# linhthi/BLISS-GNN

Hardware: AMD Instinct MI355X
Metric: steps/sec (train step: sample_blocks + gather + SAGE fwd/bwd + Adam + exp3), reddit-like (higher is better)
Workload: dtype bf16

## Files before the change

bliss_gnn_amd/_engine.py:

```python
import ctypes as C
import os
from typing import NamedTuple

import numpy as np
import torch

from . import _lib
from .graph import Block, Graph

_CHUNK = 1024
_CAP_ERRS = 1 | 2 | 4 | 8 | 64


def _ptr(t):
    return 0 if t is None else t.data_ptr()


def _stream():
    return torch.cuda.current_stream().cuda_stream


def _up8(n):
    return (int(n) + 7) & ~7

# ... 52 lines not shown
    "wlabor": _Kind("node", prob="any", entry="bliss_wlabor_layer", tail=lambda d, row: (_dep(d),) + _prob_args(d, row), p_out=True,
                    scratch=lambda e, s, b: e._scratch_grown("_wl_scr", "bliss_wlabor_scratch_bytes", s, b)),
}


class _Draw(NamedTuple):
    state: object = None
    prob: dict = None
    layer_dependency: bool = False
    iterations: int = 0


_LayerOut = NamedTuple("_LayerOut", [(name, object) for name in
                                     "indptr src dst pos eid w q kept_nid node_prob counts t_indptr t_edge".split()])


def _exact_b(rule, Eg, s, f):
    return int(min(rule.b_limit or Eg, s * f))


def layer_caps(kind, V, Eg, S0, fanouts, have=None):
    rule = KINDS[kind]
    if have is not None and len(have) != len(fanouts):
        have = None
    if have is not None and have[0]["S"] >= S0:
        if rule.k_slack is None:
            return have
        caps = [dict(c) for c in have]
    else:
        caps, s = [], int(S0)
        for f in fanouts:
            f = int(f)
            if rule.family == "layer":
                k = min(V, int(1.25 * (f + s)) + 64)
                b = int(min(Eg, max(1 << 16, 48 * k)))
            elif f < 0:
                k, b = V, int(min(Eg, max(1 << 16, 48 * s)))
            else:
                b = _exact_b(rule, Eg, s, f) if rule.b_limit is not None else int(min(Eg, 2 * s * f + 4096))
                k = int(min(V, s + min(b, Eg)))
            caps.append(dict(S=s, C=V, K=k, B=b))
            s = k
        if have is not None:
            caps = [{k: max(a.get(k, 0), b[k]) for k in b} for a, b in zip(have, caps)]
    if rule.k_slack is not None:
        for n, f in enumerate(fanouts):
            caps[n]["K"] = max(caps[n]["K"], min(V, int(f) + caps[n]["S"] + rule.k_slack))
            if n + 1 < len(caps):
                caps[n + 1]["S"] = max(caps[n + 1]["S"], caps[n]["K"])
    return have if caps == have else caps


def static_caps(kind, V, Eg, S0, fanouts, max_sizes, k_margin=1.5, b_margin=3.0):
    rule = KINDS[kind]
    caps, s = [], int(S0)
    for n, f in enumerate(fanouts):
        k = min(V, int(k_margin * max_sizes[n]["K"]) + 256)
        if rule.k_slack == 0:
            k = min(V, int(f) + s)
        b = int(min(Eg, int(b_margin * max_sizes[n]["B"]) + 4096))
        if rule.b_limit is not None and int(f) >= 0:
            b = _exact_b(rule, Eg, s, int(f))
        e = int(min(Eg, int(1.5 * max_sizes[n].get("E", Eg)) + 65536))
        x = int(min(b, int(1.5 * max_sizes[n]["B"]) + 2048))
        caps.append(dict(S=s, C=V, K=k, B=b, E=e, X=x))
        s = k
    return caps


def _parse_counts(counts_host, L):
    raw = counts_host.numpy().tobytes()
    cnts = [_lib.LayerCounts.from_buffer_copy(raw[40 * n: 40 * n + 40]) for n in range(L)]
    bad = 0
    for c in cnts:
        bad |= c.err
    return cnts, bad


class _LayerWs:

    def __init__(self, dev, cap_s, cap_c):
        self.cap_s, self.cap_c = cap_s, cap_c
        self.seg_ptr = torch.empty(cap_s + 1, dtype=torch.int32, device=dev)
        self.seed_acc = torch.empty(72 * cap_s + 64, dtype=torch.uint8, device=dev)
        self.cand_nid = torch.empty(cap_c, dtype=torch.int32, device=dev)
        self.new_id = torch.empty(cap_c, dtype=torch.int32, device=dev)
        self.p = torch.empty(cap_c, dtype=torch.bfloat16, device=dev)
        self.P = torch.empty(cap_c, dtype=torch.bfloat16, device=dev)
        self.uniforms = torch.empty(cap_c, dtype=torch.float32, device=dev)
        self.keys = torch.empty(cap_c, dtype=torch.float32, device=dev)
        self.draw_scr = torch.zeros(int(_lib.lib.bliss_multinomial_draw_scratch_bytes(cap_c)) // 4, dtype=torch.int32, device=dev)
        self.rdraw_scr = None
        self.src_cnt = None
        self.tr_temp = None


class DrawState:

    def __init__(self, seed, step, device):
        self.seed = int(seed) & ((1 << 64) - 1)
        self.step_dev = torch.tensor([int(step)], dtype=torch.int64, device=device)

    def step(self):
        return int(self.step_dev.item())


class LayerEngine:

    def __init__(self, g: Graph, kind="stream"):
        if kind not in KINDS:
            raise ValueError("kind must be one of %s, not %r" % (", ".join(KINDS), kind))
        if g.device.type != "cuda":
            raise RuntimeError("bliss_gnn_amd samples on the GPU only; move the graph with g.to('cuda') "
                               "(the reference's --data-cpu/--use-uva modes are out of scope)")
        self.g = g
        dev = g.device
        V = g.num_nodes()
        self.V, self.Eg = V, g.num_edges()
        if self.Eg >= 2 ** 31:
            raise RuntimeError("int32 edge positions: graphs with >= 2^31 edges are not supported")
        self.scratch_sets = 2
        self._sets = {}
        self.first_pos = torch.full((V,), -1, dtype=torch.int32, device=dev)
        self.acc_p2 = torch.zeros(V, dtype=torch.int64, device=dev)
        self.c_graph = _lib.Graph(g.indptr.data_ptr(), g.indices.data_ptr(), _ptr(g.eid), V, self.Eg)
        self.flags = torch.zeros(16, dtype=torch.int32, device=dev)
        self.fs_ticket = torch.zeros(1, dtype=torch.int32, device=dev)
        self.fuse_scale = os.environ.get("BLISS_FUSE_SCALE", "1") != "0"
        self.flag_err = torch.zeros(1, dtype=torch.int32, device=dev)
        self.n_bins = 0
        for nb in ((int(os.environ["BLISS_NBINS"]),) if os.environ.get("BLISS_NBINS") else (256, 1024)):
            if -(-V // nb) * 12 <= 64 * 1024:
                self.n_bins = nb
                break
        if os.environ.get("BLISS_BINS", "1") == "0" or self.Eg > 2048 * 4096 * 32:
            self.n_bins = 0
        self._bins = None
        self.hist = torch.zeros(32768, dtype=torch.int32, device=dev)
        self.mt_dev = torch.empty(626, dtype=torch.int32, device=dev)
        self.mt_host = torch.empty(626, dtype=torch.int32).pin_memory()
        self.mt_back = torch.empty(626, dtype=torch.int32).pin_memory()
        self._static = {}
        self._static_draw = {}
        self.kind = kind
        self._nr_scr = None
        self._nb_scr = None
        self._wn_scr = None
        self._lb_scr = None
        self._li_scr = None
        self._wl_scr = None
        self._wl_p = {}
        self._slot_bufs, self._slot_counts, self._slot_counts_host = {}, {}, {}
        self.caps = None
        self.ws = None
        self.counts_host = None
        self.retries = 0

    def _set(self, n):
        i = n % self.scratch_sets
        if i not in self._sets:
            dev, V = self.g.device, self.V
            local_id = torch.full((V,), -1, dtype=torch.int32, device=dev)
            self._sets[i] = dict(local_id=local_id, kept_map=torch.full((V,), -1, dtype=torch.int32, device=dev),
                                 span_seg=torch.zeros(self.Eg // 256 + 2, dtype=torch.int32, device=dev),
                                 chunk_cnt=torch.empty(max(self.Eg, V) // _CHUNK + 2, dtype=torch.int32, device=dev),
                                 kept_rec=None, span_cnt=None,
                                 c_maps=_lib.NodeMaps(local_id.data_ptr(), self.first_pos.data_ptr(), self.acc_p2.data_ptr()))
# ... 514 lines not shown
```

bliss_gnn_amd/_lib.py:

```python
import ctypes as C
import os

_HERE = os.path.dirname(os.path.abspath(__file__))
LIB_PATH = os.path.join(_HERE, "libbliss_gnn.so")

EINVAL = -1
MODE_BANDIT, MODE_LADIES, MODE_UNIFORM_NODES, MODE_PARTIALS = 0, 1, 4, 8
NR_MAX_FANOUT = 1024
WN_RAW, WN_EXP3 = 0, 1

ERR_BITS = {
    1: "frontier larger than 2^31-1 edges",
    2: "candidate capacity exceeded / seed id out of range",
    4: "kept-node capacity exceeded",
    8: "block-edge capacity exceeded",
    16: "non-finite or negative weight reached an exact reduction",
    32: "exact sum left its fixed-point range",
    64: "seed capacity exceeded",
    128: "random stream ran short / generator made no progress",
    256: "a cross-stream flag never came (bliss_flag_wait timed out)",
}


class Graph(C.Structure):
# ... 178 lines not shown
class BlockOut(C.Structure):
    _fields_ = [("indptr", C.c_void_p), ("src", C.c_void_p), ("dst", C.c_void_p), ("pos", C.c_void_p),
                ("eid", C.c_void_p), ("edge_weights", C.c_void_p), ("q_ij", C.c_void_p), ("t_indptr", C.c_void_p),
                ("t_edge", C.c_void_p), ("t_scratch", C.c_void_p), ("cap_b", C.c_int32)]


_P, _I32, _I64, _F, _D = C.c_void_p, C.c_int32, C.c_int64, C.c_float, C.c_double

SIGNATURES = {
    "bliss_layer_counts_bytes": [],
    "bliss_frontier_prob": [C.POINTER(Graph), C.POINTER(NodeMaps), _P, _P, _I32, _P, _I32, C.c_int, _F, _F, _I64, C.POINTER(LayerWs), _P],
    "bliss_rng_stream_begin": [_P, _P, _P, _P, _I32, _P],
    "bliss_rng_stream_wait": [_P, _P, _P, C.c_int, _I32, _P],
    "bliss_rng_stream_end": [_P, _P, _P, _I32, _P, _P],
    "bliss_rng_stream_chain": [_P, _P, _P, _P, _I32, _P, _I32, _P, _P],
    "bliss_rng_stream_ready": [_P],
    "bliss_rng_prepare": [_I32, _P],
    "bliss_mt_jump_poly": [_I64, _P],
    "bliss_flag_wait": [_P, _P, _P],
    "bliss_flag_set_spin_bound": [C.c_int64],
    "bliss_flag_raise": [_P, _P],
    "bliss_gather_rows": [_P, _I64, _P, _I32, _I32, _P, _I64, _P, _P],
    "bliss_exp3_apply_ranks": [C.POINTER(Exp3RankLists), _P, _P, _P, _P],
    "bliss_pack_lists": [C.POINTER(PackLists), _P, _P],
    "bliss_mt19937_uniform": [_P, _P, _I32, _P, _I32, _P],
    "bliss_poisson_select": [C.POINTER(LayerWs), _I32, _D, _P, _P, _P, C.c_int, _I32, _I64, _P],
    "bliss_poisson_select_keyed": [C.POINTER(LayerWs), _I32, _D, C.c_uint64, _P, _I32, C.c_int, _I64, _P],
    "bliss_multinomial_select": [C.POINTER(LayerWs), _P, _I32, _P],
    "bliss_multinomial_draw": [_P, _P, _P, _I32, _I32, _P, C.c_uint64, _P, _I32, C.c_int, _P, _P, _P, _P],
    "bliss_multinomial_select_marked": [C.POINTER(LayerWs), _P],
    "bliss_neighbor_layer": [C.POINTER(Graph), _P, _I32, _P, _I32, _I32, _P, C.c_uint64, _P, _I32, C.c_int, C.POINTER(LayerWs),
                             C.POINTER(BlockOut), _P, _P],
    "bliss_wneighbor_layer": [C.POINTER(Graph), _P, _I32, _P, _I32, _I32, _P, C.c_uint64, _P, _I32, C.c_int, _I32, _P, _F, _F, _P,
                              C.POINTER(LayerWs), C.POINTER(BlockOut), _P, _P],
    "bliss_neighbor_replace_layer": [C.POINTER(Graph), _P, _I32, _P, _I32, _I32, _P, C.c_uint64, _P, _I32, C.c_int, _P, _P,
                                     C.POINTER(LayerWs), C.POINTER(BlockOut), _P, _P],
    "bliss_multinomial_draw_replace": [_P, _P, _I32, _I32, _P, C.c_uint64, _P, _I32, C.c_int, _P, _P, _P, _P],
    "bliss_labor_layer": [C.POINTER(Graph), _P, _I32, _P, _I32, _I32, _P, C.c_uint64, _P, _I32, C.c_int, C.c_int, C.POINTER(LayerWs),
                          C.POINTER(BlockOut), _P, _P],
    "bliss_labor_is_layer": [C.POINTER(Graph), _P, _I32, _P, _I32, _I32, _P, C.c_uint64, _P, _I32, C.c_int, C.c_int, _I32,
                             C.POINTER(LayerWs), C.POINTER(BlockOut), _P, _P],
    "bliss_wlabor_layer": [C.POINTER(Graph), _P, _I32, _P, _I32, _I32, _P, C.c_uint64, _P, _I32, C.c_int, C.c_int, _I32, _P, _F, _F,
                           C.POINTER(LayerWs), C.POINTER(BlockOut), _P, _P, _P],
    "bliss_tile_gemm": [C.POINTER(TileGemm), C.POINTER(TileGemm), _P],
    "bliss_cross_entropy": [_P, _I64, _P, _I32, _I32, _P, _P, _I64, _P, _P, _P, _P],
    "bliss_cross_entropy_sum": [_P, _I64, _P, _I64, _P, _P, _I32, _I32, _P, _P, _I64, _P, _P, _P, _P],
    "bliss_cross_entropy_masked": [_P, _I64, _P, _I64, _P, _I32, _P, _I32, _I32, _P, _F, _I32, _P, _P, _I64, _P, _P, _P, _P],
    "bliss_cross_entropy_live": [_P, _I64, _P, _I64, _P, _P, _I32, _P, _I32, _P, _P, _I64, _P, _P, _P, _P],
    "bliss_bce_logits_live": [_P, _I64, _P, _I64, _P, _P, _I32, _P, _I32, _P, _P, _I64, _P, _P, _P, _P],
    "bliss_bce_logits": [_P, _I64, _P, _I32, _I32, _P, _P, _I64, _P, _P, _P, _P],
    "bliss_bce_logits_sum": [_P, _I64, _P, _I64, _P, _P, _I32, _I32, _P, _P, _I64, _P, _P, _P, _P],
    "bliss_bce_logits_masked": [_P, _I64, _P, _I64, _P, _I32, _P, _I32, _I32, _P, _F, _I32, _P, _P, _I64, _P, _P, _P, _P],
    "bliss_f1_multiclass": [_P, _I64, _I32, _P, _P, _P, _I32, _P, _I32, _P, _I32, _P, _P, _P],
    "bliss_f1_multilabel": [_P, _I64, _I32, _P, _P, _P, _I32, _P, _I32, _P, _I32, _P, _P, _P],
    "bliss_adam_step": [C.POINTER(AdamTensors), _P, _F, _F, _F, _F, _P],
    "bliss_step_ledger_bytes": [C.c_int],
    "bliss_step_ledger": [C.c_int, _P, C.c_int, _P, C.c_int, C.POINTER(C.c_int32), _D, _D, _P, _P],
    "bliss_batch_stats": [C.c_int, _P, C.c_int, _P, _P],
    "bliss_cand_importance": [_P, _I32, C.c_int, _P, _P, _P],
    "bliss_poisson_scale": [_P, _P, _I32, _D, _P, _P],
    "bliss_keyed_select": [_P, _P, _P, _I32, _P, C.c_uint64, C.c_uint64, _I32, _P, _P, _P],
    "bliss_exp3_normalize_global": [_P, _I64, _P, _P, _P, _P, _P],
    "bliss_build_block": [C.POINTER(Graph), C.POINTER(NodeMaps), _P, _P, _I32, C.c_int, _F, _F, _I64, C.POINTER(LayerWs), C.POINTER(BlockOut), _P],
    "bliss_normalized_edata": [C.POINTER(Graph), _P, _P],
    "bliss_embed_norm": [_P, _I32, _I32, _I64, _P, _P],
    "bliss_spmm_fwd": [_P, _P, _P, _P, _P, _I64, _I32, _P, _I32, _I32, C.c_int, _P, _I64, C.c_int, _P, _P],
    "bliss_spmm_bwd": [_P, _P, _P, _P, _P, _P, _P, _I64, _I32, _P, _I32, _I32, C.c_int, _P, _I64, C.c_int, _P, _P],
    "bliss_block_transpose": [_P, _P, _I32, _I32, _I32, _P, _P, _P, _I64, _P],
    "bliss_spmm_chunk_edges": [_I32],
    "bliss_sage_epilogue_fwd": [_P, _I64, _P, _I64, _I32, _I32, _F, C.c_uint32, _P, _P, _I64, _P, _P],
    "bliss_sage_epilogue_bwd": [_P, _I64, _P, _I64, _I32, _I32, _F, _P, _I64, _P],
    "bliss_gat_chunk_edges": [],
    "bliss_graph_prepare": [_P, _P, _I64, _I32, C.c_int, _P, _P, _P, _P, _P, _P, _I64, _P],
    "bliss_exp3_update": [C.POINTER(Graph), _P, _P, _P, _P, _P, _P, _P, _P, _P, _P, _P, _P, _I32, _P, _I32, _F, _P, _P, C.c_int, _P, _P],
    "bliss_exp3_step": [C.POINTER(Graph), _P, C.POINTER(Exp3Block), _I32, _F, _P, _P],
    "bliss_exp3_normalize_global_rows": [C.POINTER(Exp3Block), _I32, _I64, _P, _I64, _P],
    "bliss_exp3_update_blocks": [C.POINTER(Graph), _P, C.POINTER(Exp3Block), _I32, _F, _P, _P],
    "bliss_exp3_apply": [_P, _P, _P, _P, _P, _I32, _P, _P],
    "bliss_exp3_normalize": [_P, _I64, _P, _P, _P, _P],
    "bliss_row_sum": [_P, _I64, _P, _P],
    "bliss_gat_logits": [_P, _P, _P, _I32, _P, _I64, _P, _I32, _I32, _F, _P, _P],
    "bliss_sage_dgrad": [C.POINTER(DGrad), _P],
    "bliss_sage_wgrad": [C.POINTER(WGrad), _I32, _P, _I64, _P],
    "bliss_gat_dgrad": [C.POINTER(DGrad), _P],
    "bliss_gat_glue_fwd": [C.POINTER(GatGlue), _P],
    "bliss_gat_glue_bwd": [C.POINTER(GatGlue), _P],
    "bliss_gat_head_mean": [_P, _I32, _I32, _P, _P, _P],
    "bliss_gcn_norms": [_P, _I32, _P, _I32, _P, _P, _P],
    "bliss_gcn_spmm_fwd": [_P, _P, _P, _P, _P, _P, _P, _I64, _I32, _P, _I32, _I32, _P, _I64, _P, _P],
    "bliss_gcn_spmm_bwd": [_P, _P, _P, _P, _P, _P, _P, _P, _I64, _I32, _P, _I32, _I32, _P, _I64, _P, _P],
    "bliss_gcn_db_chunk_rows": [],
    "bliss_gcn_epilogue_fwd": [C.POINTER(GcnEpilogue), _P],
    "bliss_gcn_epilogue_bwd": [C.POINTER(GcnEpilogue), _P],
    "bliss_gcn_infer_chunk_edges": [_I32],
    "bliss_gcn_infer_src_norms": [C.POINTER(GcnInfer), _P],
    "bliss_gcn_infer_spmm": [C.POINTER(GcnInfer), _P],
    "bliss_shard_local_seeds": [_P, _I32, _P, _I32, _I32, _I32, _P, _P, _P, _P, _P, _P],
    "bliss_shard_scatter_partials": [_P, _P, _P, _P, _P, _P, _P, _I32, _P, _P],
    "bliss_shard_zero_dense": [_P, _I32, _P],
    "bliss_shard_pack_rows": [_P, _P, _I32, _I32, _I32, _P, _I64, _I32, _P, _I64, _P],
    "bliss_shard_place_rows": [_P, _I64, _P, _P, _I32, _P, _I64, _I32, _I32, _P],
    "bliss_shard_take_rows": [_P, _I32, _I64, _I32, _P, _P, _I32, _P, _I64, _I32, _P],
    "bliss_shard_candidates": [_P, _I32, _I32, _P, _P, _P, _P, _P, _I32, _P, _P, _P],
    "bliss_shard_select_kept": [_P, _P, _P, _P, C.c_uint64, _P, _I32, _P, _I32, _P, _P, _P, _P, _P, _I32, _I32, _I32, _P, _P, _P, _I32, _P, _P, _P],
    "bliss_gat_fused_supported": [_I32, _I32],
    "bliss_gat_segment_edges": [],
    "bliss_gat_fused_stamps": [_P, _P],
    "bliss_gat_segments": [_P, _I32, _I32, _P, _P, _P, _P],
    "bliss_gat_fused_fwd": [C.POINTER(GatFused), _P],
    "bliss_gat_fused_bwd_dst": [C.POINTER(GatFused), _P, _P, _P, _P],
    "bliss_gat_infer_fwd": [C.POINTER(GatInfer), _P],
    "bliss_gat_rows_src_fused": [_P, _I32, _P, _P, _P, _P, _I32, _P, _P, _P, _I64, _P, _I64, _P, _I32, _I32, _F, _P, _I64, _P, _P],
    "bliss_gat_logits_f32": [_P, _P, _P, _I32, _P, _I64, _P, _I32, _I32, _F, _P, _P],
    "bliss_gat_edge_dot": [_P, _P, _P, _I32, _P, _I64, _P, _I64, _I32, _I32, _P, _P],
    "bliss_gat_edge_softmax": [_P, _I32, _P, _P, _I32, C.c_int, _P, _P],
    "bliss_gat_rows": [C.c_int, _P, _I32, _P, _P, _P, _P, _I32, _P, _P, _I64, _P, _I32, _I32, _F, _P, _I64, _P, _P, _P],
    "bliss_gat_alpha": [_P, _I32, _P, _P, _P, _P, _P],
    "bliss_prof_enable": [C.c_int],
    "bliss_prof_reset": [],
    "bliss_prof_read": [C.c_int, C.POINTER(C.c_double), C.POINTER(C.c_int64)],
    "bliss_prof_kernel_count": [],
}


SPECIAL_SIGNATURES = ("bliss_prof_kernel_name", "bliss_block_transpose_temp_bytes", "bliss_graph_prepare_capacity",
                      "bliss_graph_prepare_temp_bytes", "bliss_rng_stream_handle", "bliss_sage_wgrad_workspace",
                      "bliss_multinomial_draw_scratch_bytes", "bliss_neighbor_scratch_bytes", "bliss_wneighbor_scratch_bytes",
                      "bliss_labor_scratch_bytes", "bliss_labor_is_scratch_bytes", "bliss_wlabor_scratch_bytes",
                      "bliss_neighbor_replace_scratch_bytes", "bliss_multinomial_draw_replace_scratch_bytes")


def _load():
    if not os.path.exists(LIB_PATH):
        raise ImportError(
            f"{LIB_PATH} not found: build it with `python -c 'import __graft_entry__ as g; g.build()'` "
            "or `make -C bliss_gnn_amd/csrc`.  bliss_gnn_amd has no CPU or PyTorch fallback.")
    lib = C.CDLL(LIB_PATH)
    for name, argtypes in SIGNATURES.items():
        fn = getattr(lib, name)
        fn.argtypes = argtypes
        fn.restype = C.c_int
    lib.bliss_block_transpose_temp_bytes.argtypes = [_I32, _I32]
    lib.bliss_block_transpose_temp_bytes.restype = C.c_int64
    lib.bliss_sage_wgrad_workspace.argtypes = [C.POINTER(WGrad), _I32]
    lib.bliss_sage_wgrad_workspace.restype = C.c_int64
    for name in ("bliss_graph_prepare_capacity", "bliss_graph_prepare_temp_bytes"):
        getattr(lib, name).argtypes = [_I64, _I32, C.c_int]
        getattr(lib, name).restype = C.c_int64
    lib.bliss_multinomial_draw_scratch_bytes.argtypes = [_I32]
    lib.bliss_multinomial_draw_scratch_bytes.restype = C.c_int64
    lib.bliss_neighbor_scratch_bytes.argtypes = [_I32, _I32]
    lib.bliss_neighbor_scratch_bytes.restype = C.c_int64
    lib.bliss_wneighbor_scratch_bytes.argtypes = [_I32, _I32, _I64]
    lib.bliss_wneighbor_scratch_bytes.restype = C.c_int64
    lib.bliss_labor_scratch_bytes.argtypes = [_I32, _I32]
    lib.bliss_labor_scratch_bytes.restype = C.c_int64
    lib.bliss_labor_is_scratch_bytes.argtypes = [_I32, _I32, _I32]
    lib.bliss_labor_is_scratch_bytes.restype = C.c_int64
    lib.bliss_wlabor_scratch_bytes.argtypes = [_I32, _I32, _I32]
    lib.bliss_wlabor_scratch_bytes.restype = C.c_int64
    lib.bliss_neighbor_replace_scratch_bytes.argtypes = [_I32, _I32]
    lib.bliss_neighbor_replace_scratch_bytes.restype = C.c_int64
    lib.bliss_multinomial_draw_replace_scratch_bytes.argtypes = [_I32]
    lib.bliss_multinomial_draw_replace_scratch_bytes.restype = C.c_int64
    lib.bliss_rng_stream_handle.argtypes = []
    lib.bliss_rng_stream_handle.restype = C.c_int64
    lib.bliss_prof_kernel_name.argtypes = [C.c_int]
    lib.bliss_prof_kernel_name.restype = C.c_char_p
    assert lib.bliss_layer_counts_bytes() == C.sizeof(LayerCounts), "LayerCounts layout mismatch"
    assert all(lib.bliss_step_ledger_bytes(n) == C.sizeof(ledger_struct(n)) for n in range(1, LEDGER_MAX_LAYERS + 1)), \
        "step ledger layout mismatch"
    assert C.sizeof(BatchStats) == 32, "batch statistics layout mismatch"
    return lib


lib = _load()


def check(rc, what):
    if rc != 0:
        raise RuntimeError(f"{what} failed with code {rc}" + (" (invalid argument)" if rc == EINVAL else " (hipError_t)"))


def err_string(bits):
    return "; ".join(msg for b, msg in ERR_BITS.items() if bits & b) or "unknown"
```

bliss_gnn_amd/csrc/sage_bwd.hip:

```cpp
#include "common.cuh"
#include "bliss_gnn.h"
#include <cstdlib>

namespace {

typedef __bf16 bf16x8_t __attribute__((ext_vector_type(8)));
typedef short s16x4_t __attribute__((ext_vector_type(4)));
typedef short s16x8_t __attribute__((ext_vector_type(8)));
typedef float f32x16_t __attribute__((ext_vector_type(16)));
typedef uint32_t u32x4_a4 __attribute__((ext_vector_type(4), aligned(4)));

__device__ __forceinline__ s16x4_t lds_tr4(const bf16_t* p) {
  return __builtin_amdgcn_ds_read_tr16_b64_v4i16((__attribute__((address_space(3))) s16x4_t*)(p));
}
__device__ __forceinline__ bf16x8_t tr_frag(const bf16_t* img, int stride, int k0, int c0, int lane) {
  const int g = lane >> 4, i = lane & 15, q = i >> 2, p = i & 3;
  const bf16_t* a = img + (size_t)(k0 + 8 * (g >> 1) + q) * stride + c0 + 16 * (g & 1) + 4 * p;
  const s16x4_t lo = lds_tr4(a), hi = lds_tr4(a + 4 * (size_t)stride);
  s16x8_t v;
  v[0] = lo[0]; v[1] = lo[1]; v[2] = lo[2]; v[3] = lo[3]; v[4] = hi[0]; v[5] = hi[1]; v[6] = hi[2]; v[7] = hi[3];
  return __builtin_bit_cast(bf16x8_t, v);
}

__device__ __forceinline__ uint4 ld16(const bf16_t* p) {
// ... 41 lines not shown
    *reinterpret_cast<uint4*>(wl + (size_t)kr * DG_WSTRIDE + 8 * c8) = v;
  }
}

__device__ __forceinline__ void dg_product(const bf16_t* tile, int k, const bf16_t* __restrict__ w, long long w_stride, int N, int n0,
                                           bf16_t* wl, int tid, int lane, int wave, f32x16_t& acc) {
  const int st = dg_astride(k), kp = (k + 15) & ~15, r = lane & 31, h = lane >> 5;
  const int nslab = (kp + DG_SLAB - 1) / DG_SLAB;
  for (int sl = 0; sl < nslab; ++sl) {
    __syncthreads();
    dg_stage_w(w, w_stride, k, N, n0, sl, wl, tid);
    __syncthreads();
#pragma unroll
    for (int s = 0; s < DG_SLAB / 16; ++s) {
      const int ks = sl * DG_SLAB + 16 * s;
      if (ks < kp) {
        const bf16x8_t a = *reinterpret_cast<const bf16x8_t*>(tile + (size_t)r * st + ks + 8 * h);
        const bf16x8_t b = tr_frag(wl, DG_WSTRIDE, 16 * s, 32 * wave, lane);
        acc = __builtin_amdgcn_mfma_f32_32x32x16_bf16(a, b, acc, 0, 0, 0);
      }
    }
  }
}

__global__ void __launch_bounds__(DG_TPB) k_dgrad(DGrad p) {
  extern __shared__ __attribute__((aligned(16))) bf16_t dg_lds[];
  const int tid = threadIdx.x, wave = tid >> 6, lane = tid & 63;
  int M = p.m_bound;
  if (p.m_dev) { const int t = *p.m_dev; M = t < M ? t : M; }
  int M2 = p.k2 ? p.m2_bound : 0;
  if (p.k2 && p.m2_dev) { const int t = *p.m2_dev; M2 = t < M2 ? t : M2; }
  if (M2 > M) M2 = M;
  const int row0 = blockIdx.x * DG_M, n0 = blockIdx.y * 256, N = p.n;
  if (row0 >= p.m_bound) return;
  const bool pair_ok = (p.out_stride % 2 == 0) && (((uintptr_t)p.out) % 4 == 0) && (N % 2 == 0);
  if (row0 >= M) {
    for (int idx = tid; idx < DG_M * 256; idx += DG_TPB) {
      const int r = row0 + (idx >> 8), c = n0 + (idx & 255);
      if (r < p.m_bound && c < N) p.out[(long long)r * p.out_stride + c] = 0;
    }
    return;
  }
  const int s1 = dg_astride(p.k1), s2 = p.k2 ? dg_astride(p.k2) : 0;
  bf16_t* t1 = dg_lds;
  bf16_t* t2 = t1 + (size_t)DG_M * s1;
  bf16_t* wl = t2 + (size_t)DG_M * s2;
  dg_stage_a(p.a1, p.a1_stride, p.k1, row0, M, t1, tid);
  const bool second = p.k2 && row0 < M2;
  if (second) dg_stage_a(p.a2, p.a2_stride, p.k2, row0, M2, t2, tid);
  f32x16_t acc;
#pragma unroll
  for (int i = 0; i < 16; ++i) acc[i] = 0.f;
  dg_product(t1, p.k1, p.w1, p.w1_stride, N, n0, wl, tid, lane, wave, acc);
  if (second) dg_product(t2, p.k2, p.w2, p.w2_stride, N, n0, wl, tid, lane, wave, acc);
  __syncthreads();
  const int so = 256 + 8;
  bf16_t* ot = dg_lds;
  {
    const int col = 32 * wave + (lane & 31);
#pragma unroll
    for (int i = 0; i < 16; ++i) {
      const int lr = (i & 3) + 8 * (i >> 2) + 4 * (lane >> 5);
      ot[(size_t)lr * so + col] = (row0 + lr < M) ? f2bf(acc[i]) : (bf16_t)0;
    }
  }
  __syncthreads();
  for (int lr = wave; lr < DG_M; lr += DG_TPB / 64) {
    const int r = row0 + lr;
    if (r >= p.m_bound) break;
    const bf16_t* sh = ot + (size_t)lr * so;
    bf16_t* o = p.out + (long long)r * p.out_stride + n0;
    const int nn = min(256, N - n0);
    if (pair_ok && (n0 % 2 == 0)) { for (int c = lane * 2; c < nn; c += 128) *reinterpret_cast<uint32_t*>(o + c) = *reinterpret_cast<const uint32_t*>(sh + c); }
    else for (int c = lane; c < nn; c += 64) o[c] = sh[c];
  }
}

#define WG_TPB 512
#define WG_ROWS 32
#define WG_TN 128
#define WG_DSTRIDE (256 + 32)
#define WG_XSTRIDE (WG_TN + 32)
#define WG_MAX_PROBS 2

struct WGradProb {
  const bf16_t* d; long long d_stride; int n_out;
  const bf16_t* x; long long x_stride; int k_in;
  int rows_bound; const int* rows_dev;
  bf16_t* dw; long long dw_stride; bf16_t* db;
  int col_tiles, chunks, rows_per_chunk; long long part_off;
  int ldp;
  int wg_begin;
};
struct WGradLaunch { WGradProb p[WG_MAX_PROBS]; int n; };

struct WRegsB { uint4 d[2]; uint4 x; };

__device__ __forceinline__ void wg_load(WRegsB& g, const WGradProb& p, int r_lo, int r_hi, int c0, int tid, bool d_al, bool x_al) {
#pragma unroll
  for (int i = 0; i < 2; ++i) {
    const int idx = tid + i * WG_TPB, lr = idx >> 5, c8 = idx & 31, r = r_lo + lr, n = 8 * c8;
    g.d[i] = (r < r_hi) ? ld8_masked(p.d + (long long)r * p.d_stride + n, p.n_out - n, d_al) : make_uint4(0, 0, 0, 0);
  }
  {
    const int lr = tid >> 4, c8 = tid & 15, r = r_lo + lr, c = c0 + 8 * c8;
    g.x = (r < r_hi) ? ld8_masked(p.x + (long long)r * p.x_stride + c, p.k_in - c, x_al) : make_uint4(0, 0, 0, 0);
  }
}
__device__ __forceinline__ void wg_store(const WRegsB& g, bf16_t* dimg, bf16_t* ximg, int tid) {
#pragma unroll
  for (int i = 0; i < 2; ++i) {
    const int idx = tid + i * WG_TPB, lr = idx >> 5, c8 = idx & 31;
    *reinterpret_cast<uint4*>(dimg + (size_t)lr * WG_DSTRIDE + 8 * c8) = g.d[i];
  }
  *reinterpret_cast<uint4*>(ximg + (size_t)(tid >> 4) * WG_XSTRIDE + 8 * (tid & 15)) = g.x;
}

__global__ void __launch_bounds__(WG_TPB) k_wgrad(WGradLaunch L, float* __restrict__ part) {
  __shared__ __attribute__((aligned(16))) bf16_t dimg[WG_ROWS * WG_DSTRIDE];
  __shared__ __attribute__((aligned(16))) bf16_t ximg[WG_ROWS * WG_XSTRIDE];
  const int tid = threadIdx.x, wave = tid >> 6, lane = tid & 63;
  const int pi = (L.n > 1 && (int)blockIdx.x >= L.p[1].wg_begin) ? 1 : 0;
  const WGradProb& p = L.p[pi];
  const int w = (int)blockIdx.x - p.wg_begin;
  const int ct = w % p.col_tiles, ch = w / p.col_tiles;
  int R = p.rows_bound;
  if (p.rows_dev) { const int t = *p.rows_dev; R = t < R ? t : R; }
  const int r_lo = ch * p.rows_per_chunk, r_hi = min(R, r_lo + p.rows_per_chunk);
  if (r_lo >= r_hi) return;
  const int c0 = ct * WG_TN;
  const int wm = wave >> 1, wn = wave & 1;
  const int m0 = 64 * wm, nl0 = 64 * wn;
  const bool m_act = m0 < p.n_out;
  const bool bias = p.db != nullptr && ct == 0 && wn == 0;
  f32x16_t acc[2][2], accb[2];
#pragma unroll
  for (int a = 0; a < 2; ++a) {
#pragma unroll
    for (int i = 0; i < 16; ++i) { acc[a][0][i] = 0.f; acc[a][1][i] = 0.f; accb[a][i] = 0.f; }
  }
  s16x8_t ones_s;
#pragma unroll
  for (int j = 0; j < 8; ++j) ones_s[j] = (short)0x3f80;
  const bf16x8_t ones = __builtin_bit_cast(bf16x8_t, ones_s);
  const bool d_al = (p.d_stride % 2 == 0) && (((uintptr_t)p.d) % 4 == 0);
  const bool x_al = (p.x_stride % 2 == 0) && (((uintptr_t)p.x) % 4 == 0);
  WRegsB g;
  wg_load(g, p, r_lo, r_hi, c0, tid, d_al, x_al);
  for (int rs = r_lo; rs < r_hi; rs += WG_ROWS) {
    __syncthreads();
    wg_store(g, dimg, ximg, tid);
    if (rs + WG_ROWS < r_hi) wg_load(g, p, rs + WG_ROWS, r_hi, c0, tid, d_al, x_al);
    __syncthreads();
    if (m_act) {
#pragma unroll
      for (int ks = 0; ks < WG_ROWS; ks += 16) {
        const bf16x8_t a0 = tr_frag(dimg, WG_DSTRIDE, ks, m0, lane), a1 = tr_frag(dimg, WG_DSTRIDE, ks, m0 + 32, lane);
        const bf16x8_t b0 = tr_frag(ximg, WG_XSTRIDE, ks, nl0, lane), b1 = tr_frag(ximg, WG_XSTRIDE, ks, nl0 + 32, lane);
        acc[0][0] = __builtin_amdgcn_mfma_f32_32x32x16_bf16(a0, b0, acc[0][0], 0, 0, 0);
        acc[0][1] = __builtin_amdgcn_mfma_f32_32x32x16_bf16(a0, b1, acc[0][1], 0, 0, 0);
        acc[1][0] = __builtin_amdgcn_mfma_f32_32x32x16_bf16(a1, b0, acc[1][0], 0, 0, 0);
        acc[1][1] = __builtin_amdgcn_mfma_f32_32x32x16_bf16(a1, b1, acc[1][1], 0, 0, 0);
        if (bias) {
          accb[0] = __builtin_amdgcn_mfma_f32_32x32x16_bf16(a0, ones, accb[0], 0, 0, 0);
          accb[1] = __builtin_amdgcn_mfma_f32_32x32x16_bf16(a1, ones, accb[1], 0, 0, 0);
        }
      }
    }
  }
  if (!m_act) return;
  float* pt = part + p.part_off + (long long)ch * 256 * p.ldp;
#pragma unroll
  for (int a = 0; a < 2; ++a) {
#pragma unroll
    for (int i = 0; i < 16; ++i) {
      const int n = m0 + 32 * a + (i & 3) + 8 * (i >> 2) + 4 * (lane >> 5);
      float* row = pt + (long long)n * p.ldp;
      row[c0 + nl0 + (lane & 31)] = acc[a][0][i];
      row[c0 + nl0 + 32 + (lane & 31)] = acc[a][1][i];
      if (bias && (lane & 31) == 0) row[p.col_tiles * WG_TN] = accb[a][i];
    }
  }
}

__global__ void __launch_bounds__(256) k_wgrad_reduce(WGradLaunch L, const float* __restrict__ part) {
  const int pi = blockIdx.y;
  const WGradProb& p = L.p[pi];
  int R = p.rows_bound;
  if (p.rows_dev) { const int t = *p.rows_dev; R = t < R ? t : R; }
  const int nch = R > 0 ? min(p.chunks, (R + p.rows_per_chunk - 1) / p.rows_per_chunk) : 0;
  const int q4 = (p.k_in + 3) / 4 + (p.db ? 1 : 0);
  const long long total = (long long)p.n_out * q4;
  const float* base = part + p.part_off;
  for (long long idx = (long long)blockIdx.x * 256 + threadIdx.x; idx < total; idx += (long long)gridDim.x * 256) {
    const int n = (int)(idx / q4), q = (int)(idx - (long long)n * q4);
    if (p.db && q == q4 - 1) {
      float s = 0.f;
      for (int c = 0; c < nch; ++c) s += base[((long long)c * 256 + n) * p.ldp + p.col_tiles * WG_TN];
      p.db[n] = f2bf(s);
      continue;
    }
    float4 s = make_float4(0.f, 0.f, 0.f, 0.f);
    for (int c = 0; c < nch; ++c) {
      const float4 v = *reinterpret_cast<const float4*>(base + ((long long)c * 256 + n) * p.ldp + 4 * q);
      s.x += v.x; s.y += v.y; s.z += v.z; s.w += v.w;
    }
    bf16_t* o = p.dw + (long long)n * p.dw_stride + 4 * q;
    const int left = p.k_in - 4 * q;
    o[0] = f2bf(s.x);
    if (left > 1) o[1] = f2bf(s.y);
    if (left > 2) o[2] = f2bf(s.z);
    if (left > 3) o[3] = f2bf(s.w);
  }
}

int wgrad_target_wgs() {
  static const int t = []() { const char* e = getenv("BLISS_WGRAD_WGS"); const int v = e ? atoi(e) : 0; return v > 0 ? v : 80; }();
  return t;
}

bool wgrad_plan(const bliss_wgrad_t* a, int n_probs, WGradLaunch* L, long long* floats, int* total_wgs) {
  if (n_probs < 1 || n_probs > WG_MAX_PROBS) return false;
  long long off = 0;
  int wgs = 0;
  int tiles_all = 0;
  for (int i = 0; i < n_probs; ++i) {
    if (!a[i].d || !a[i].x || !a[i].dw || a[i].n_out <= 0 || a[i].n_out > 256 || a[i].k_in <= 0 || a[i].rows_bound <= 0) return false;
    tiles_all += (a[i].k_in + WG_TN - 1) / WG_TN;
  }
  for (int i = 0; i < n_probs; ++i) {
    WGradProb& p = L->p[i];
    p.d = (const bf16_t*)a[i].d; p.d_stride = a[i].d_stride; p.n_out = a[i].n_out;
    p.x = (const bf16_t*)a[i].x; p.x_stride = a[i].x_stride; p.k_in = a[i].k_in;
    p.rows_bound = a[i].rows_bound; p.rows_dev = a[i].rows_dev;
    p.dw = (bf16_t*)a[i].dw; p.dw_stride = a[i].dw_stride; p.db = (bf16_t*)a[i].db;
    p.col_tiles = (a[i].k_in + WG_TN - 1) / WG_TN;
    int chunks = wgrad_target_wgs() / tiles_all;
    const int max_chunks = (a[i].rows_bound + 63) / 64;
    if (chunks > max_chunks) chunks = max_chunks;
    if (chunks < 1) chunks = 1;
    int rpc = (a[i].rows_bound + chunks - 1) / chunks;
    rpc = (rpc + WG_ROWS - 1) / WG_ROWS * WG_ROWS;
    chunks = (a[i].rows_bound + rpc - 1) / rpc;
    p.chunks = chunks; p.rows_per_chunk = rpc;
    p.ldp = p.col_tiles * WG_TN + 4;
    p.part_off = off;
    p.wg_begin = wgs;
    off += (long long)chunks * 256 * p.ldp;
    wgs += chunks * p.col_tiles;
  }
  L->n = n_probs;
  *floats = off;
  *total_wgs = wgs;
  return true;
}

int dgrad_launch(const bliss_dgrad_t* a, int k_max, void* stream) {
  if (!a || !a->a1 || !a->w1 || !a->out || a->k1 <= 0 || a->k1 > k_max || a->n <= 0 || a->m_bound <= 0) return BLISS_EINVAL;
  if (a->k2 < 0 || a->k2 > k_max || (a->k2 > 0 && (!a->a2 || !a->w2 || a->m2_bound <= 0))) return BLISS_EINVAL;
  DGrad p;
  p.a1 = (const bf16_t*)a->a1; p.a1_stride = a->a1_stride; p.w1 = (const bf16_t*)a->w1; p.w1_stride = a->w1_stride; p.k1 = a->k1;
  p.a2 = (const bf16_t*)a->a2; p.a2_stride = a->a2_stride; p.w2 = (const bf16_t*)a->w2; p.w2_stride = a->w2_stride; p.k2 = a->k2;
  p.m2_bound = a->m2_bound; p.m2_dev = a->m2_dev;
  p.m_bound = a->m_bound; p.m_dev = a->m_dev; p.n = a->n;
  p.out = (bf16_t*)a->out; p.out_stride = a->out_stride;
  const size_t stage = ((size_t)DG_M * (dg_astride(a->k1) + (a->k2 ? dg_astride(a->k2) : 0)) + (size_t)DG_SLAB * DG_WSTRIDE) * sizeof(bf16_t);
  const size_t outt = (size_t)DG_M * (256 + 8) * sizeof(bf16_t);
  const size_t lds = stage > outt ? stage : outt;
  if (lds > 160 * 1024) return BLISS_EINVAL;
  static size_t lds_set = 0;
  if (lds > lds_set) {
    if (hipFuncSetAttribute((const void*)k_dgrad, hipFuncAttributeMaxDynamicSharedMemorySize, (int)lds) != hipSuccess) return BLISS_EINVAL;
    lds_set = lds;
  }
  const dim3 grid((a->m_bound + DG_M - 1) / DG_M, (a->n + 255) / 256);
  k_dgrad<<<grid, DG_TPB, lds, (hipStream_t)stream>>>(p);
  return (int)hipGetLastError();
}

}

extern "C" {

int bliss_sage_dgrad(const bliss_dgrad_t* a, void* stream) { return dgrad_launch(a, 256, stream); }

int bliss_gat_dgrad(const bliss_dgrad_t* a, void* stream) { return dgrad_launch(a, 1024, stream); }

int64_t bliss_sage_wgrad_workspace(const bliss_wgrad_t* probs, int32_t n_probs) {
  WGradLaunch L;
  long long floats = 0;
  int wgs = 0;
  if (!probs || !wgrad_plan(probs, n_probs, &L, &floats, &wgs)) return -1;
  return (int64_t)floats;
}

int bliss_sage_wgrad(const bliss_wgrad_t* probs, int32_t n_probs, float* partials, int64_t partial_floats, void* stream) {
  WGradLaunch L;
  long long floats = 0;
  int wgs = 0;
  if (!probs || !partials || !wgrad_plan(probs, n_probs, &L, &floats, &wgs)) return BLISS_EINVAL;
  if (partial_floats < floats || (((uintptr_t)partials) % 16) != 0) return BLISS_EINVAL;
  hipStream_t st = (hipStream_t)stream;
  k_wgrad<<<wgs, WG_TPB, 0, st>>>(L, partials);
  int max_elems = 0;
  for (int i = 0; i < n_probs; ++i) { const int e = L.p[i].n_out * ((L.p[i].k_in + 3) / 4 + 1); if (e > max_elems) max_elems = e; }
  int gx = (max_elems + 255) / 256;
  if (gx > 1024) gx = 1024;
  k_wgrad_reduce<<<dim3(gx, n_probs), 256, 0, st>>>(L, partials);
  return (int)hipGetLastError();
}

}
```

bliss_gnn_amd/csrc/sampler.hip:

```cpp
#include "common.cuh"
#include "bliss_gnn.h"
#include "prof.h"
#include "edge_q.cuh"
#include "keyed_uniform.cuh"
#include <cstdlib>

#ifndef TPB
#define TPB 256
#endif
#define ITEMS 4
#define CHUNK (TPB * ITEMS)

namespace {

#define SPAN (64 * ITEMS)
#define SEG_ZERO_WGS 8
#define LONG_COL 1024
#define LONG_FIRST 4096

struct alignas(8) ColEnt {
  int k, n;
  long long p0;
};

struct EdgeAt {
  int k;
  int64_t pos;
  int src;
};

__device__ __forceinline__ EdgeAt decode(int base, int E, int S, const int* __restrict__ seg_ptr,
                                         const long long* __restrict__ col_base, const int* __restrict__ indices, int* k_hint) {
  EdgeAt r;
  const int e = base + lane_id();
  r.k = wave_segment(seg_ptr, S, base, k_hint);
  r.pos = 0; r.src = 0;
  if (e < E) {
    r.pos = col_base[r.k] + e;
    r.src = indices[r.pos];
  } else r.k = -1;
  return r;
}

struct SpanAt {
  int k[ITEMS];
  int64_t pos[ITEMS];
  int src[ITEMS];
};
__device__ __forceinline__ bool decode_span(int wbase, int E, int S, const int* __restrict__ seg_ptr,
                                            const long long* __restrict__ col_base, const int* __restrict__ indices, int k_hint,
                                            SpanAt& r) {
  k_hint = k_hint < 0 ? 0 : (k_hint < S ? k_hint : S - 1);
  if (!span_segments<ITEMS>(seg_ptr, S, wbase, E - 1, k_hint, r.k)) return false;
  long long cb[ITEMS];
#pragma unroll
  for (int j = 0; j < ITEMS; ++j) cb[j] = col_base[r.k[j]];
#pragma unroll
  for (int j = 0; j < ITEMS; ++j) {
    const int e = wbase + j * 64 + lane_id();
    r.pos[j] = cb[j] + (e < E ? e : E - 1);
    r.src[j] = indices[r.pos[j]];
  }
  return true;
}

__device__ __forceinline__ int chunk_wave_offset(int wave_total, int* sh4, int* chunk_total) {
  const int wave = threadIdx.x >> 6;
  __syncthreads();
  if (lane_id() == 0) sh4[wave] = wave_total;
  __syncthreads();
  int off = 0, tot = 0;
#pragma unroll
  for (int w = 0; w < TPB / 64; ++w) { const int v = sh4[w]; tot += v; if (w < wave) off += v; }
  *chunk_total = tot;
  return off;
}

__device__ __forceinline__ void seg_scan_body(const int64_t* __restrict__ indptr, const int* __restrict__ seeds,
                                              LayerCounts* cnt, int S_host, const int* __restrict__ S_dev, int cap_s,
                                              unsigned long long* __restrict__ seed_acc, int* __restrict__ seg_ptr,
                                              int* __restrict__ local_id, int num_nodes, int* __restrict__ src_cnt, int cap_k,
                                              int* __restrict__ bin_cursor, int n_bins, long long* __restrict__ col_base,
                                              int* __restrict__ span_seg, long long frontier_cap, int* entry_flag,
                                              int wg, int n_wgs, bool keep_sums, int* sh, int* st_sh, ColEnt* long_list = nullptr) {
  if (entry_flag && wg == 0 && threadIdx.x == 0) __hip_atomic_store(entry_flag, 1, __ATOMIC_RELEASE, __HIP_MEMORY_SCOPE_AGENT);
  __shared__ int sh_long[2];
  if (long_list && threadIdx.x < 2) sh_long[threadIdx.x] = 0;
  int S = S_host >= 0 ? S_host : *S_dev;
  int bad = 0;
  if (S > cap_s) { S = cap_s; bad |= BLISS_ERR_CAP_SEEDS; }
  if (wg > 0 || n_wgs == 1) {
    const int nz = n_wgs > 1 ? n_wgs - 1 : 1, bz = n_wgs > 1 ? wg - 1 : 0;
    const int t0 = bz * blockDim.x + threadIdx.x, step = nz * blockDim.x;
    for (int i = (keep_sums ? 2 * cap_s : 0) + t0; i < cap_s * 5; i += step) seed_acc[i] = 0ull;
    if (src_cnt) for (int i = t0; i <= cap_k; i += step) src_cnt[i] = 0;
    if (bin_cursor) for (int i = t0; i <= n_bins; i += step) bin_cursor[i] = 0;
    for (int k = t0; k < S; k += step) { const int s = seeds[k]; if (s >= 0 && s < num_nodes) local_id[s] = k; }
    if (n_wgs > 1) return;
  }
  long long run = 0;
  constexpr int G = 4;
  for (int base0 = 0; base0 < S; base0 += G * (int)blockDim.x) {
    int degs[G];
    long long cols[G];
#pragma unroll
    for (int i = 0; i < G; ++i) {
      const int k = base0 + i * (int)blockDim.x + threadIdx.x;
      degs[i] = 0; cols[i] = 0;
      if (k < S) {
        const int s = seeds[k];
        if (s < 0 || s >= num_nodes) { bad |= BLISS_ERR_CAP_CAND; }
        else {
          cols[i] = indptr[s];
          degs[i] = (int)(indptr[s + 1] - cols[i]);
        }
      }
    }
#pragma unroll
    for (int i = 0; i < G; ++i) {
      const int k = base0 + i * (int)blockDim.x + threadIdx.x;
      if (base0 + i * (int)blockDim.x >= S) break;
      const int deg = degs[i];
      int tot, ex = block_excl_scan(deg, sh, &tot);
      const long long start = run + ex;
      if (k < S) {
        seg_ptr[k] = (int)start;
        col_base[k] = deg > 0 ? cols[i] - start : 0;
      }
      if (long_list) {
        const bool is_long = k < S && deg > LONG_COL, is_first = is_long && deg > LONG_FIRST;
        const unsigned long long m_first = __ballot(is_first), m_rest = __ballot(is_long && !is_first);
        if (m_first | m_rest) {
          int b_first = 0, b_rest = 0;
          if (lane_id() == 0) {
            if (m_first) b_first = atomicAdd(&sh_long[0], __popcll(m_first));
            if (m_rest) b_rest = atomicAdd(&sh_long[1], __popcll(m_rest));
          }
          b_first = __shfl(b_first, 0); b_rest = __shfl(b_rest, 0);
          if (is_long) {
            const unsigned long long below = (1ull << lane_id()) - 1ull;
            const int slot = is_first ? b_first + __popcll(m_first & below) : cap_s - 1 - (b_rest + __popcll(m_rest & below));
            ColEnt ent; ent.k = k; ent.n = deg; ent.p0 = cols[i];
            long_list[slot] = ent;
          }
        }
      }
      if (run + tot <= frontier_cap) {
        st_sh[threadIdx.x] = (int)(k < S ? start : run + tot);
        __syncthreads();
        const long long sp_end = (run + tot + SPAN - 1) / SPAN;
        for (long long sp = (run + SPAN - 1) / SPAN + threadIdx.x; sp < sp_end; sp += blockDim.x) {
          const int p = (int)(sp * SPAN);
          int t = 0;
#pragma unroll
          for (int step = 512; step >= 1; step >>= 1) if (st_sh[t + step] <= p) t += step;
          span_seg[sp] = base0 + i * (int)blockDim.x + t;
        }
      }
      run += tot;
      if (run > frontier_cap) bad |= BLISS_ERR_CAP_FRONTIER;
    }
  }
  int any_bad = __syncthreads_or(bad);
  if (threadIdx.x == 0) {
    if (long_list) { int* n_long = (int*)(long_list + cap_s); n_long[0] = sh_long[0]; n_long[1] = sh_long[1]; }
    seg_ptr[S] = (int)run;
    cnt->S = S; cnt->E = (any_bad & BLISS_ERR_CAP_FRONTIER) ? 0 : (int)run;
    cnt->C = 0; cnt->K = 0; cnt->B = 0; cnt->iters = 0; cnt->all_one = 0; cnt->c = 1.0;
    cnt->err = any_bad;
  }
}

__global__ void __launch_bounds__(1024) k_seg_scan(const int64_t* __restrict__ indptr, const int* __restrict__ seeds,
                                                   LayerCounts* cnt, int S_host, const int* __restrict__ S_dev, int cap_s,
                                                   unsigned long long* __restrict__ seed_acc, int* __restrict__ seg_ptr,
                                                   int* __restrict__ local_id, int num_nodes, int* __restrict__ src_cnt, int cap_k,
                                                   int* __restrict__ bin_cursor, int n_bins, long long* __restrict__ col_base,
                                                   int* __restrict__ span_seg, long long frontier_cap, int* entry_flag,
                                                   int keep_sums, ColEnt* long_list) {
  __shared__ int sh[17];
  __shared__ int st_sh[1024];
  seg_scan_body(indptr, seeds, cnt, S_host, S_dev, cap_s, seed_acc, seg_ptr, local_id, num_nodes, src_cnt, cap_k, bin_cursor, n_bins,
                col_base, span_seg, frontier_cap, entry_flag, blockIdx.x, gridDim.x, keep_sums != 0, sh, st_sh, long_list);
}

template <bool BANDIT>
__global__ void __launch_bounds__(TPB) k_frontier_pass1(const int64_t* __restrict__ indptr, const int* __restrict__ indices,
                                                        const bf16_t* __restrict__ w, const int* __restrict__ seeds,
                                                        const int* __restrict__ seg_ptr, const long long* __restrict__ col_base,
    const int* __restrict__ span_seg, LayerCounts* cnt,
                                                        const int* __restrict__ local_id, unsigned* first_pos,
                                                        unsigned long long* acc_w) {
  const int S = cnt->S, E = cnt->E;
  const int nspans = (E + SPAN - 1) / SPAN;
  int bad = 0;
  for (int sp = blockIdx.x * (TPB / 64) + (threadIdx.x >> 6); sp < nspans; sp += gridDim.x * (TPB / 64)) {
    int hint = span_seg[sp];
#pragma unroll
    for (int i = 0; i < ITEMS; ++i) {
      const int base = sp * SPAN + i * 64;
      if (base >= E) break;
      const int e = base + lane_id();
      EdgeAt a = decode(base, E, S, seg_ptr, col_base, indices, &hint);
      int64_t term = 0;
      if (a.k >= 0) {
        if (local_id[a.src] < 0) {
          if (__hip_atomic_load(first_pos + a.src, __ATOMIC_RELAXED, __HIP_MEMORY_SCOPE_AGENT) > (unsigned)e)
            atomicMin(first_pos + a.src, (unsigned)e);
        }
        if (BANDIT) term = bf_to_fixed(w[a.pos], FRAC_DST, &bad);
      }
      if (BANDIT) wave_segsum_atomic_i64(a.k, term, acc_w);
    }
  }
  if (bad) atomicOr(&cnt->err, bad);
}

template <bool BANDIT>
__global__ void __launch_bounds__(TPB) k_frontier_pass2(const int64_t* __restrict__ indptr, const int* __restrict__ indices,
                                                        const bf16_t* __restrict__ w, const int* __restrict__ seeds,
                                                        const int* __restrict__ seg_ptr, const long long* __restrict__ col_base,
    const int* __restrict__ span_seg, LayerCounts* cnt,
                                                        const unsigned* __restrict__ first_pos,
                                                        const unsigned long long* __restrict__ acc_w,
                                                        unsigned long long* acc_q, int* __restrict__ chunk_cnt,
                                                        float eta_f, float ome_f) {
  __shared__ int sh4[TPB / 64];
  const int S = cnt->S, E = cnt->E;
  const int nchunks = (E + CHUNK - 1) / CHUNK;
  int bad = 0;
  for (int chunk = blockIdx.x; chunk < nchunks; chunk += gridDim.x) {
    int nfirst = 0, hint = span_seg[chunk * ITEMS + (threadIdx.x >> 6)];
#pragma unroll
    for (int i = 0; i < ITEMS; ++i) {
      const int base = chunk * CHUNK + (threadIdx.x >> 6) * SPAN + i * 64;
      if (base >= E) break;
      const int e = base + lane_id();
      EdgeAt a = decode(base, E, S, seg_ptr, col_base, indices, &hint);
      int64_t term = 0;
      bool first = false;
      if (a.k >= 0) {
        first = first_pos[a.src] == (unsigned)e;
        if (BANDIT) {
          bf16_t wsum = fixed_to_bf((int64_t)acc_w[a.k], FRAC_DST, &bad);
          bf16_t q = edge_q(w[a.pos], wsum, seg_ptr[a.k + 1] - seg_ptr[a.k], eta_f, ome_f);
          term = bf_to_fixed(q, FRAC_DST, &bad);
        }
      }
      nfirst += __popcll(__ballot(first));
      if (BANDIT) wave_segsum_atomic_i64(a.k, term, acc_q);
    }
    int tot;
    chunk_wave_offset(nfirst, sh4, &tot);
    if (threadIdx.x == 0) chunk_cnt[chunk] = tot;
  }
  if (bad) atomicOr(&cnt->err, bad);
}

__global__ void __launch_bounds__(1024) k_chunk_scan(int* __restrict__ chunk_cnt, LayerCounts* cnt, int which, int cap) {
  __shared__ int sh[17];
  int n_items = which == 1 ? cnt->C : cnt->E;
  const int n = (n_items + CHUNK - 1) / CHUNK;
  int run = 0;
  for (int base = 0; base < n; base += blockDim.x) {
    int i = base + threadIdx.x;
    int v = i < n ? chunk_cnt[i] : 0;
// ... 58 lines not shown
      mask[i] = __ballot(first);
      wave_total += __popcll(mask[i]);
    }
    int tot;
    int run = S + chunk_off[chunk] + chunk_wave_offset(wave_total, sh4, &tot);
#pragma unroll
    for (int i = 0; i < ITEMS; ++i) {
      if ((mask[i] >> lane_id()) & 1ull) {
        const int id = run + __popcll(mask[i] & ((1ull << lane_id()) - 1ull));
        if (id < cap_c) { local_id[srcs[i]] = id; cand_nid[id] = srcs[i]; }
      }
      run += __popcll(mask[i]);
    }
  }
  if (bad) atomicOr(&cnt->err, bad);
}

#define HIST_BINS 32768
#define HWIN_LO 0x3000
#define HWIN_N 4096
#ifndef FIN_TPB
#define FIN_TPB 1024
#endif
__global__ void __launch_bounds__(FIN_TPB) k_cand_finalize(const int* __restrict__ seeds, LayerCounts* cnt, int* __restrict__ cand_nid,
                                                           unsigned long long* acc_p2, unsigned* first_pos,
                                                           bf16_t* __restrict__ p, int* hist, int cap_c, int uniform_nodes) {
  __shared__ int lh[HIST_BINS];
  const int S = cnt->S;
  const int C = min(cnt->C, cap_c);
  if ((int)blockIdx.x * FIN_TPB >= C) return;
  {
    int4* lh4 = reinterpret_cast<int4*>(lh);
    for (int b = threadIdx.x; b < HIST_BINS / 4; b += FIN_TPB) lh4[b] = make_int4(0, 0, 0, 0);
  }
  __syncthreads();
  int bad = 0;
  for (int id = blockIdx.x * FIN_TPB + threadIdx.x; id < C; id += gridDim.x * FIN_TPB) {
    int g;
    if (id < S) { g = seeds[id]; cand_nid[id] = g; } else g = cand_nid[id];
    const unsigned long long raw = acc_p2[g];
    acc_p2[g] = 0;
    first_pos[g] = 0xffffffffu;
    bf16_t pj;
    if (uniform_nodes) pj = raw ? (bf16_t)0x3f80 : (bf16_t)0;
    else pj = f2bf(sqrtf(bf2f(fixed_to_bf((int64_t)raw, FRAC_SRC, &bad))));
    p[id] = pj;
    if (pj < HIST_BINS) atomicAdd(&lh[pj], 1); else bad |= BLISS_ERR_NONFINITE;
  }
  __syncthreads();
  {
    const int4* lh4 = reinterpret_cast<const int4*>(lh);
    for (int b = threadIdx.x; b < HIST_BINS / 4; b += FIN_TPB) {
      const int4 v = lh4[b];
      if (v.x | v.y | v.z | v.w) {
        if (v.x) atomicAdd(hist + 4 * b, v.x);
        if (v.y) atomicAdd(hist + 4 * b + 1, v.y);
        if (v.z) atomicAdd(hist + 4 * b + 2, v.z);
        if (v.w) atomicAdd(hist + 4 * b + 3, v.w);
      }
    }
  }
  if (bad) atomicOr(&cnt->err, bad);
}

#define BIN_TPB 1024
#ifndef BIN_ITEMS
#define BIN_ITEMS 4
#endif
#define BIN_BATCH (BIN_TPB * BIN_ITEMS)
#define MAX_BINS 1024
#ifndef COL_TPB
#define COL_TPB 1024
#endif
#ifndef COL_R
#define COL_R 16
#endif
#ifndef COL_RB
#define COL_RB 8
#endif
#ifndef COL_BLOCK_WGS
#define COL_BLOCK_WGS 512
#endif
#define COL_BIG (COL_R * 64)
static_assert(LONG_COL == COL_BIG, "k_seg_scan lists the columns k_col_sums treats as long");
#ifndef BINRED_TPB
#define BINRED_TPB 1024
#endif

template <int NT>
__device__ __forceinline__ int block_max_u31(int v, long long* sh) {
  v = wave_max_u31(v);
  __syncthreads();
  if (lane_id() == 0) sh[threadIdx.x >> 6] = v;
  __syncthreads();
  int t = 0;
#pragma unroll
  for (int w = 0; w < NT / 64; ++w) t = max(t, (int)sh[w]);
  return t;
}

template <int NT>
__device__ __forceinline__ long long block_sum2_i64(long long a, long long b, long long* sh2, long long* b_out) {
  a = wave_total_i64(a);
  b = wave_total_i64(b);
  __syncthreads();
  if (lane_id() == 0) { sh2[threadIdx.x >> 6] = a; sh2[NT / 64 + (threadIdx.x >> 6)] = b; }
  __syncthreads();
  long long ta = 0, tb = 0;
#pragma unroll
  for (int w = 0; w < NT / 64; ++w) { ta += sh2[w]; tb += sh2[NT / 64 + w]; }
  *b_out = tb;
  return ta;
}

template <int NT>
__device__ __forceinline__ long long block_sum_i64(long long v, long long* sh) {
  v = wave_total_i64(v);
  __syncthreads();
  if (lane_id() == 0) sh[threadIdx.x >> 6] = v;
  __syncthreads();
  long long t = 0;
#pragma unroll
  for (int w = 0; w < NT / 64; ++w) t += sh[w];
  return t;
}

template <int N>
struct PackedBf {
  unsigned v[N / 2];
  __device__ __forceinline__ void set(int r, bf16_t x) { v[r >> 1] = (r & 1) ? (v[r >> 1] | ((unsigned)x << 16)) : (unsigned)x; }
  __device__ __forceinline__ bf16_t get(int r) const { return (bf16_t)((r & 1) ? v[r >> 1] >> 16 : v[r >> 1] & 0xffffu); }
};

__device__ __forceinline__ const bf16_t* uniform_ptr(const bf16_t* p) {
  const unsigned long long v = (unsigned long long)p;
  const unsigned lo = __builtin_amdgcn_readfirstlane((int)(unsigned)v), hi = __builtin_amdgcn_readfirstlane((int)(unsigned)(v >> 32));
  return (const bf16_t*)(((unsigned long long)hi << 32) | lo);
}

__device__ __forceinline__ void col_store(int k, long long ws_fixed, long long qs_fixed, bf16_t wsum, int n, float eta_f,
                                          unsigned long long* acc_w, unsigned long long* acc_q, uint2* seed_coef, int* bad) {
  acc_w[k] = (unsigned long long)ws_fixed; acc_q[k] = (unsigned long long)qs_fixed;
  const bf16_t qsum = fixed_to_bf(qs_fixed, FRAC_DST, bad);
  seed_coef[k] = make_uint2((unsigned)wsum | ((unsigned)qsum << 16), __float_as_uint(rbf((1.0f / (float)n) * eta_f)));
}

__global__ void __launch_bounds__(COL_TPB, 8) k_col_sums(const int64_t* __restrict__ indptr, const bf16_t* __restrict__ w,
                                                      const int* __restrict__ seeds, const int* __restrict__ seg_ptr,
                                                      const long long* __restrict__ col_base, const int* __restrict__ span_seg,
                                                      LayerCounts* cnt, unsigned long long* __restrict__ acc_w,
                                                      unsigned long long* __restrict__ acc_q, float eta_f, float ome_f,
                                                      uint2* __restrict__ seed_coef, int n_block_wgs,
                                                      const ColEnt* __restrict__ long_list, int cap_s) {
  __shared__ long long sh[COL_TPB / 64];
  __shared__ long long sh2[2 * COL_TPB / 64];
  const int tid = threadIdx.x, lane = lane_id();
  const int* n_long = (const int*)(long_list + cap_s);
  const int S = cnt->S, E = cnt->E, n_first = n_long[0], n_all = n_first + n_long[1];
  if (E == 0) return;
  int bad = 0;
  const int bid_wave = (int)blockIdx.x, bid_block = (int)blockIdx.x - ((int)gridDim.x - n_block_wgs);
  if (bid_block < 0) {
  const int k = bid_wave * (COL_TPB / 64) + __builtin_amdgcn_readfirstlane(tid >> 6);
  const int s0 = k < S ? seg_ptr[k] : 0, n = k < S ? seg_ptr[k + 1] - s0 : 0;
  const long long cb = k < S ? col_base[k] : 0;
  if (n > 0 && n <= COL_BIG) {
    const bf16_t* wc = uniform_ptr(w + (cb + s0));
    PackedBf<COL_R> wr;
    long long part = 0;
    int emax = 1;
    {
      bf16_t x[COL_R];
#pragma unroll
      for (int r = 0; r < COL_R; ++r) {
        const int i = lane + r * 64;
        x[r] = 0;
        if (i < n) x[r] = wc[i];
      }
#pragma unroll
      for (int r = 0; r < COL_R; ++r) wr.set(r, x[r]);
    }
#pragma unroll
    for (int r = 0; r < COL_R; ++r)
      if (lane + r * 64 < n) emax = max(emax, bf_exp_field(wr.get(r)));
    const int wfrac = rel_frac(FRAC_DST, wave_max_u31(emax));
    const PlainRange wr_ok = bf_plain_range(wfrac);
    bool odd = false;
#pragma unroll
    for (int r = 0; r < COL_R; ++r)
      if (r * 64 < n) {
        odd |= lane + r * 64 < n && !bf_is_plain(wr.get(r), wr_ok);
        part += bf_fixed_plain(wr.get(r), wfrac);
      }
    long long ws_fixed;
    bf16_t wsum;
    if (__ballot(odd) == 0ull) {
      ws_fixed = wave_total_i64(part);
      wsum = fixed_to_bf(ws_fixed, wfrac, &bad);
    } else {
      long long part_lo = 0;
      int sticky = 0;
      part = 0;
#pragma unroll 4
      for (int i = lane; i < n; i += 64) part += bf_to_fixed_wide(wc[i], wfrac, &part_lo, &sticky, &bad);
      ws_fixed = wave_total_i64(part);
      if (__ballot(part_lo != 0 || sticky) == 0ull) wsum = fixed_to_bf(ws_fixed, wfrac, &bad);
      else wsum = fixed_wide_to_bf(ws_fixed, wave_total_i64(part_lo), __ballot(sticky) != 0ull, wfrac, &bad);
    }
    const float a = rbf((1.0f / (float)n) * eta_f);
    const PlainRange q_ok = bf_plain_range(FRAC_DST);
    part = 0; odd = false;
#pragma unroll
    for (int r = 0; r < COL_R; ++r)
      if (r * 64 < n) {
        const bool in = lane + r * 64 < n;
        const bf16_t q = edge_q_pre(wr.get(r), wsum, a, ome_f);
        odd |= in && !bf_is_plain(q, q_ok);
        part += in ? bf_fixed_plain(q, FRAC_DST) : 0ll;
      }
    if (__ballot(odd) != 0ull) {
      part = 0;
#pragma unroll 4
      for (int i = lane; i < n; i += 64) part += bf_to_fixed(edge_q_pre(wc[i], wsum, a, ome_f), FRAC_DST, &bad);
    }
    const long long qs_fixed = wave_total_i64(part);
    if (lane == 0) col_store(k, ws_fixed, qs_fixed, wsum, n, eta_f, acc_w, acc_q, seed_coef, &bad);
  }
  }
  if (bid_block >= 0) {
  for (int li = bid_block; li < n_all; li += n_block_wgs) {
    const ColEnt ent = long_list[li < n_first ? li : cap_s - 1 - (li - n_first)];
    const int k = ent.k, n = ent.n;
    const bf16_t* wc = uniform_ptr(w + ent.p0);
    int t = tid;
    asm volatile("" : "+v"(t));
    const int wave0 = __builtin_amdgcn_readfirstlane(t & ~63);
    PackedBf<COL_RB> wr;
    long long part = 0;
    int emax = 1;
    {
      bf16_t x[COL_RB];
#pragma unroll
      for (int r = 0; r < COL_RB; ++r) {
        const int i = t + r * COL_TPB;
        x[r] = 0;
        if (i < n) x[r] = wc[i];
      }
#pragma unroll
      for (int r = 0; r < COL_RB; ++r) wr.set(r, x[r]);
    }
#pragma unroll
    for (int r = 0; r < COL_RB; ++r)
      if (t + r * COL_TPB < n) emax = max(emax, bf_exp_field(wr.get(r)));
#pragma unroll 8
    for (int i = t + COL_RB * COL_TPB; i < n; i += COL_TPB) emax = max(emax, bf_exp_field(wc[i]));
    const int wfrac = rel_frac(FRAC_DST, block_max_u31<COL_TPB>(emax, sh));
    const PlainRange wr_ok = bf_plain_range(wfrac);
    bool odd = false;
#pragma unroll
    for (int r = 0; r < COL_RB; ++r)
      if (wave0 + r * COL_TPB < n) {
        odd |= t + r * COL_TPB < n && !bf_is_plain(wr.get(r), wr_ok);
        part += bf_fixed_plain(wr.get(r), wfrac);
      }
#pragma unroll 8
    for (int i = t + COL_RB * COL_TPB; i < n; i += COL_TPB) {
      const bf16_t b = wc[i];
      odd |= !bf_is_plain(b, wr_ok);
      part += bf_fixed_plain(b, wfrac);
    }
    long long lost;
    long long ws_fixed = block_sum2_i64<COL_TPB>(part, odd ? 1 : 0, sh2, &lost);
    bf16_t wsum;
    if (lost == 0) wsum = fixed_to_bf(ws_fixed, wfrac, &bad);
    else {
      long long part_lo = 0;
      int sticky = 0;
      part = 0;
#pragma unroll 4
      for (int i = t; i < n; i += COL_TPB) part += bf_to_fixed_wide(wc[i], wfrac, &part_lo, &sticky, &bad);
      ws_fixed = block_sum2_i64<COL_TPB>(part, (part_lo != 0 || sticky) ? 1 : 0, sh2, &lost);
      if (lost == 0) wsum = fixed_to_bf(ws_fixed, wfrac, &bad);
      else {
        const long long lo_tot = block_sum_i64<COL_TPB>(part_lo, sh);
        const long long st_tot = block_sum_i64<COL_TPB>(sticky, sh);
        wsum = fixed_wide_to_bf(ws_fixed, lo_tot, st_tot != 0, wfrac, &bad);
      }
    }
    const float a = rbf((1.0f / (float)n) * eta_f);
    const PlainRange q_ok = bf_plain_range(FRAC_DST);
    part = 0; odd = false;
#pragma unroll
    for (int r = 0; r < COL_RB; ++r)
      if (wave0 + r * COL_TPB < n) {
        const bool in = t + r * COL_TPB < n;
        const bf16_t q = edge_q_pre(wr.get(r), wsum, a, ome_f);
        odd |= in && !bf_is_plain(q, q_ok);
        part += in ? bf_fixed_plain(q, FRAC_DST) : 0ll;
      }
#pragma unroll 8
    for (int i = t + COL_RB * COL_TPB; i < n; i += COL_TPB) {
      const bf16_t q = edge_q_pre(wc[i], wsum, a, ome_f);
      odd |= !bf_is_plain(q, q_ok);
      part += bf_fixed_plain(q, FRAC_DST);
    }
    long long qs_fixed = block_sum2_i64<COL_TPB>(part, odd ? 1 : 0, sh2, &lost);
    if (lost != 0) {
      part = 0;
#pragma unroll 4
      for (int i = t; i < n; i += COL_TPB) part += bf_to_fixed(edge_q_pre(wc[i], wsum, a, ome_f), FRAC_DST, &bad);
      qs_fixed = block_sum_i64<COL_TPB>(part, sh);
    }
    if (t == 0) col_store(k, ws_fixed, qs_fixed, wsum, n, eta_f, acc_w, acc_q, seed_coef, &bad);
  }
  }
  if (bad) atomicOr(&cnt->err, bad);
}

template <bool BANDIT>
__global__ void __launch_bounds__(BIN_TPB) k_bin_scatter(const int64_t* __restrict__ indptr, const int* __restrict__ indices,
                                                     const bf16_t* __restrict__ w, const int* __restrict__ seeds,
                                                     const int* __restrict__ seg_ptr, const long long* __restrict__ col_base,
    const int* __restrict__ span_seg, LayerCounts* cnt,
                                                     const unsigned long long* __restrict__ acc_w,
                                                     const unsigned long long* __restrict__ acc_q, float eta_f, float ome_f,
                                                     int uniform_nodes, int n_bins, int log2_bins, long long bin_cap, int* bin_cursor,
                                                     unsigned long long* __restrict__ bin_rec, unsigned* __restrict__ bitmap,
                                                     const uint2* __restrict__ seed_coef) {
  __shared__ int hist[MAX_BINS];
  __shared__ int gbase[MAX_BINS];
  const int S = cnt->S, E = cnt->E, tid = threadIdx.x;
  const int nb = (E + BIN_BATCH - 1) / BIN_BATCH;
  const int bmask = n_bins - 1;
  int bad = 0;
  for (int batch = blockIdx.x; batch < nb; batch += gridDim.x) {
    for (int b = tid; b < n_bins; b += BIN_TPB) hist[b] = 0;
    if (tid < BIN_BATCH / 32) bitmap[batch * (BIN_BATCH / 32) + tid] = 0u;
    __syncthreads();
    int srcs[BIN_ITEMS], ranks[BIN_ITEMS];
    bf16_t ts[BIN_ITEMS];
    const int wbase = batch * BIN_BATCH + (tid >> 6) * (64 * BIN_ITEMS);
    int hint = span_seg[wbase >> 8];
    SpanAt sp;
    if (wbase < E && decode_span(wbase, E, S, seg_ptr, col_base, indices, hint, sp)) {
      bf16_t wv[BIN_ITEMS];
      uint2 cf[BIN_ITEMS];
      if (!uniform_nodes) {
#pragma unroll
        for (int j = 0; j < BIN_ITEMS; ++j) {
          wv[j] = w[sp.pos[j]];
          if (BANDIT) cf[j] = seed_coef[sp.k[j]];
        }
      }
#pragma unroll
      for (int j = 0; j < BIN_ITEMS; ++j) {
        bf16_t t;
        if (uniform_nodes) {
          t = (bf16_t)0x3f80;
        } else if (BANDIT) {
          bf16_t q = edge_q_pre(wv[j], (bf16_t)(cf[j].x & 0xffffu), __uint_as_float(cf[j].y), ome_f);
          float r = rbf(bf2f(q) / bf2f((bf16_t)(cf[j].x >> 16)));
          t = f2bf(r * r);
        } else {
          float x = bf2f(wv[j]);
          t = f2bf(x * x);
        }
        srcs[j] = sp.src[j]; ts[j] = t;
        ranks[j] = wbase + j * 64 + lane_id() < E ? atomicAdd(&hist[sp.src[j] & bmask], 1) : -1;
      }
    } else {
#pragma unroll
    for (int j = 0; j < BIN_ITEMS; ++j) {
      ranks[j] = -1; srcs[j] = 0; ts[j] = 0;
      const int base = wbase + j * 64;
      if (base >= E) continue;
      EdgeAt a = decode(base, E, S, seg_ptr, col_base, indices, &hint);
      if (a.k >= 0) {
        bf16_t t;
        if (uniform_nodes) {
          t = (bf16_t)0x3f80;
        } else if (BANDIT) {
          const uint2 cf = seed_coef[a.k];
          bf16_t q = edge_q_pre(w[a.pos], (bf16_t)(cf.x & 0xffffu), __uint_as_float(cf.y), ome_f);
          float r = rbf(bf2f(q) / bf2f((bf16_t)(cf.x >> 16)));
          t = f2bf(r * r);
        } else {
          float x = bf2f(w[a.pos]);
          t = f2bf(x * x);
        }
        srcs[j] = a.src; ts[j] = t;
        ranks[j] = atomicAdd(&hist[a.src & bmask], 1);
      }
    }
    }
    __syncthreads();
    for (int b = tid; b < n_bins; b += BIN_TPB) {
      const int h = hist[b];
      int g0 = 0;
      if (h) {
        g0 = atomicAdd(bin_cursor + b, h);
        if ((long long)g0 + h > bin_cap) bad |= BLISS_ERR_CAP_CAND;
      }
      gbase[b] = g0;
    }
    __syncthreads();
#pragma unroll
    for (int j = 0; j < BIN_ITEMS; ++j) {
      if (ranks[j] >= 0) {
        const int b = srcs[j] & bmask;
        const long long idx = (long long)gbase[b] + ranks[j];
        if (idx < bin_cap) {
          const size_t o = (size_t)b * (size_t)bin_cap + (size_t)idx;
          const unsigned e = (unsigned)(wbase + j * 64 + lane_id());
          bin_rec[o] = ((unsigned long long)e << 32) | ((unsigned long long)((unsigned)srcs[j] >> log2_bins) << 15) | (ts[j] & 0x7fffu);
// ... 716 lines not shown
  maps_cleanup(cnt, cand_nid, local_id, cap_c, kept_nid, kept_map, cap_k);
}

inline int grid_for(int64_t n, int per_block, int max_blocks = 8192) {
  int64_t g = (n + per_block - 1) / per_block;
  if (g < 1) g = 1;
  if (g > max_blocks) g = max_blocks;
  return (int)g;
}

}

#define CK(x) do { hipError_t e_ = (x); if (e_ != hipSuccess) return (int)e_; } while (0)

static long long g_flag_spin_bound = 1ll << 22;
__global__ void __launch_bounds__(64) k_flag_wait(int* flag, int* err, long long bound) {
  if (threadIdx.x != 0) return;
  long long spins = 0;
  while (__hip_atomic_load(flag, __ATOMIC_RELAXED, __HIP_MEMORY_SCOPE_AGENT) == 0) {
    __builtin_amdgcn_s_sleep(8);
    if (++spins > bound) { if (err) atomicOr(err, BLISS_ERR_FLAG_TIMEOUT); break; }
  }
  __builtin_amdgcn_fence(__ATOMIC_ACQUIRE, "agent");
  __hip_atomic_store(flag, 0, __ATOMIC_RELAXED, __HIP_MEMORY_SCOPE_AGENT);
}

__global__ void k_flag_raise(int* flag) {
  if (threadIdx.x == 0) __hip_atomic_store(flag, 1, __ATOMIC_RELEASE, __HIP_MEMORY_SCOPE_AGENT);
}

extern "C" {

int bliss_layer_counts_bytes(void) { return (int)sizeof(LayerCounts); }

int bliss_flag_raise(int32_t* flag, void* stream) {
  if (!flag) return BLISS_EINVAL;
  k_flag_raise<<<1, 64, 0, (hipStream_t)stream>>>(flag);
  return (int)hipGetLastError();
}

int bliss_flag_wait(int32_t* flag, int32_t* err_word, void* stream) {
  if (!flag) return BLISS_EINVAL;
  k_flag_wait<<<1, 64, 0, (hipStream_t)stream>>>(flag, err_word, g_flag_spin_bound);
  return (int)hipGetLastError();
}

int bliss_flag_set_spin_bound(int64_t spins) {
  if (spins < 1) return BLISS_EINVAL;
  g_flag_spin_bound = spins;
  return 0;
}

int bliss_frontier_prob(const bliss_graph_t* g, const bliss_node_maps_t* m, const void* w_pos, const int32_t* seeds,
                        int32_t n_seeds, const int32_t* n_seeds_dev, int32_t cap_s, int mode, float eta_f,
                        float one_minus_eta_f, int64_t frontier_bound, const bliss_layer_ws_t* ws, void* stream_) {
  if (!g || !m || !seeds || !ws || !w_pos || cap_s <= 0 || !ws->hist || !ws->span_seg) return BLISS_EINVAL;
  if (n_seeds < 0 && !n_seeds_dev) return BLISS_EINVAL;
  if (n_seeds > cap_s) return BLISS_EINVAL;
  const int uniform_nodes = (mode & BLISS_MODE_UNIFORM_NODES) ? 1 : 0;
  const bool partials_only = (mode & BLISS_MODE_PARTIALS) != 0;
  mode &= ~(BLISS_MODE_UNIFORM_NODES | BLISS_MODE_PARTIALS);
  if (mode != BLISS_MODE_BANDIT && mode != BLISS_MODE_LADIES) return BLISS_EINVAL;
  if (partials_only && ws->n_bins <= 0) return BLISS_EINVAL;
  hipStream_t st = (hipStream_t)stream_;
  LayerCounts* cnt = (LayerCounts*)ws->counts;
  const bf16_t* w = (const bf16_t*)w_pos;
  unsigned long long* acc_w = (unsigned long long*)ws->seed_acc;
  unsigned long long* acc_q = acc_w + cap_s;
  const long long* col_base = (const long long*)(acc_w + 5 * (size_t)cap_s);
  if (frontier_bound < 1) frontier_bound = 1;
  const int ge = grid_for(frontier_bound, TPB), gc = grid_for(frontier_bound, CHUNK);
  const bool binned = ws->n_bins > 0;
  int log2_bins = 0, slots = 0;
  if (binned) {
    while ((1 << log2_bins) < ws->n_bins) ++log2_bins;
    slots = (g->num_nodes + ws->n_bins - 1) >> log2_bins;
    if ((1 << log2_bins) != ws->n_bins || ws->n_bins > MAX_BINS || (size_t)slots * 12 > 64 * 1024 || ws->bin_cap <= 0 ||
        g->num_edges > (long long)MAX_TILES * BTILE * 32 || !ws->bin_cursor || !ws->bin_rec || !ws->bitmap || !ws->word_prefix || !ws->touched_key || !ws->touched_sum)
      return BLISS_EINVAL;
  }
  const long long fcap = (long long)(g->num_edges < 0x7fffffffll ? g->num_edges : 0x7fffffffll);
  const bool col_sums = binned && mode == BLISS_MODE_BANDIT;
  ColEnt* long_list = (ColEnt*)(acc_w + 7 * (size_t)cap_s);
  PROF_LAUNCH(BK_SEG_SCAN, st, k_seg_scan<<<1 + SEG_ZERO_WGS, 1024, 0, st>>>(g->indptr, seeds, cnt, n_seeds, n_seeds_dev, cap_s, acc_w, ws->seg_ptr,
                                                            m->local_id, g->num_nodes, ws->src_cnt, ws->cap_k,
                                                            binned ? ws->bin_cursor : nullptr, ws->n_bins, (long long*)col_base, ws->span_seg,
                                                            fcap, ws->entry_flag, col_sums ? 1 : 0, col_sums ? long_list : nullptr));
  if (binned) {
    unsigned long long* seed_p2 = acc_w + 4 * (size_t)cap_s;
    uint2* seed_coef = (uint2*)(acc_w + 6 * (size_t)cap_s);
    unsigned long long* bin_rec = (unsigned long long*)ws->bin_rec;
    const int gb = grid_for(frontier_bound, BIN_BATCH);
    const int n_wave_wgs = (cap_s + COL_TPB / 64 - 1) / (COL_TPB / 64), n_block_wgs = cap_s < COL_BLOCK_WGS ? cap_s : COL_BLOCK_WGS;
    if (col_sums)
      PROF_LAUNCH(BK_COL_SUMS, st, k_col_sums<<<n_block_wgs + n_wave_wgs, COL_TPB, 0, st>>>(g->indptr, w, seeds, ws->seg_ptr, col_base, ws->span_seg, cnt, acc_w, acc_q, eta_f, one_minus_eta_f, seed_coef, n_block_wgs, long_list, cap_s));
    if (mode == BLISS_MODE_BANDIT)
      PROF_LAUNCH(BK_BIN_SCATTER, st, k_bin_scatter<true><<<gb, BIN_TPB, 0, st>>>(g->indptr, g->indices, w, seeds, ws->seg_ptr, col_base, ws->span_seg, cnt, acc_w, acc_q, eta_f, one_minus_eta_f, uniform_nodes, ws->n_bins, log2_bins, ws->bin_cap, ws->bin_cursor, bin_rec, ws->bitmap, seed_coef));
    else
      PROF_LAUNCH(BK_BIN_SCATTER, st, k_bin_scatter<false><<<gb, BIN_TPB, 0, st>>>(g->indptr, g->indices, w, seeds, ws->seg_ptr, col_base, ws->span_seg, cnt, acc_w, acc_q, eta_f, one_minus_eta_f, uniform_nodes, ws->n_bins, log2_bins, ws->bin_cap, ws->bin_cursor, bin_rec, ws->bitmap, seed_coef));
    PROF_LAUNCH(BK_BIN_REDUCE, st, k_bin_reduce<<<ws->n_bins, BINRED_TPB, (size_t)slots * 12, st>>>(
        cnt, ws->n_bins, log2_bins, ws->bin_cap, ws->bin_cursor, bin_rec, g->num_nodes, slots, m->local_id, seed_p2,
        (unsigned long long*)ws->touched_key, (unsigned long long*)ws->touched_sum, ws->bitmap, ws->cap_c));
    if (partials_only) return (int)hipGetLastError();
    int* tile_sum = ws->word_prefix;
    int* word_prefix = ws->word_prefix + MAX_TILES;
    PROF_LAUNCH(BK_BITMAP_SCAN, st, k_bitmap_tiles<<<grid_for(frontier_bound, (int64_t)BTILE * 32, MAX_TILES), 1024, 0, st>>>(ws->bitmap, word_prefix, tile_sum, cnt));
    int gf = (ws->cap_c + FIN_TPB - 1) / FIN_TPB;
    if (gf < 1) gf = 1;
    if (gf > 512) gf = 512;
    PROF_LAUNCH(BK_CAND_NUMBER, st, k_cand_number<<<gf, FIN_TPB, 0, st>>>(
        seeds, cnt, ws->cand_nid, m->local_id, seed_p2, (const unsigned long long*)ws->touched_key,
        (const unsigned long long*)ws->touched_sum, ws->bitmap, word_prefix, tile_sum, (bf16_t*)ws->p, ws->hist, ws->cap_c, uniform_nodes,
        FusedScale{ws->fs_ticket, ws->fs_fanout, ws->fs_eps, ws->fs_rng_ctl, ws->fs_layer_off, ws->fs_is_last, ws->fs_rng_cap, ws->chunk_cnt}));
    return (int)hipGetLastError();
  }
  if (mode == BLISS_MODE_BANDIT) {
    PROF_LAUNCH(BK_PASS1, st, k_frontier_pass1<true><<<ge, TPB, 0, st>>>(g->indptr, g->indices, w, seeds, ws->seg_ptr, col_base, ws->span_seg, cnt, m->local_id, m->first_pos, acc_w));
    PROF_LAUNCH(BK_PASS2, st, k_frontier_pass2<true><<<gc, TPB, 0, st>>>(g->indptr, g->indices, w, seeds, ws->seg_ptr, col_base, ws->span_seg, cnt, m->first_pos, acc_w, acc_q, ws->chunk_cnt, eta_f, one_minus_eta_f));
  } else {
    PROF_LAUNCH(BK_PASS1, st, k_frontier_pass1<false><<<ge, TPB, 0, st>>>(g->indptr, g->indices, w, seeds, ws->seg_ptr, col_base, ws->span_seg, cnt, m->local_id, m->first_pos, acc_w));
    PROF_LAUNCH(BK_PASS2, st, k_frontier_pass2<false><<<gc, TPB, 0, st>>>(g->indptr, g->indices, w, seeds, ws->seg_ptr, col_base, ws->span_seg, cnt, m->first_pos, acc_w, acc_q, ws->chunk_cnt, eta_f, one_minus_eta_f));
  }
  PROF_LAUNCH(BK_CHUNK_SCAN, st, k_chunk_scan<<<1, 1024, 0, st>>>(ws->chunk_cnt, cnt, 0, ws->cap_c));
  if (mode == BLISS_MODE_BANDIT)
    PROF_LAUNCH(BK_PASS3, st, k_frontier_pass3<true><<<gc, TPB, 0, st>>>(g->indptr, g->indices, w, seeds, ws->seg_ptr, col_base, ws->span_seg, cnt, m->first_pos, acc_w, acc_q, ws->chunk_cnt, m->local_id, ws->cand_nid, (unsigned long long*)m->acc_p2, eta_f, one_minus_eta_f, ws->cap_c, uniform_nodes));
  else
    PROF_LAUNCH(BK_PASS3, st, k_frontier_pass3<false><<<gc, TPB, 0, st>>>(g->indptr, g->indices, w, seeds, ws->seg_ptr, col_base, ws->span_seg, cnt, m->first_pos, acc_w, acc_q, ws->chunk_cnt, m->local_id, ws->cand_nid, (unsigned long long*)m->acc_p2, eta_f, one_minus_eta_f, ws->cap_c, uniform_nodes));
  {
    int gf = (ws->cap_c + FIN_TPB * 8 - 1) / (FIN_TPB * 8);
    if (gf < 1) gf = 1;
    if (gf > 256) gf = 256;
    PROF_LAUNCH(BK_CAND_FINALIZE, st, k_cand_finalize<<<gf, FIN_TPB, 0, st>>>(
        seeds, cnt, ws->cand_nid, (unsigned long long*)m->acc_p2, m->first_pos, (bf16_t*)ws->p, ws->hist, ws->cap_c, uniform_nodes));
  }
  return (int)hipGetLastError();
}

int bliss_poisson_select(const bliss_layer_ws_t* ws, int32_t fanout, double eps, const float* uniforms,
                         int32_t* uniforms_offset_dev, int32_t* rng_ctl, int is_last, int32_t rng_cap_total,
                         int64_t cand_bound, void* stream_) {
  if (!ws || !uniforms || fanout < 0 || (rng_ctl && !uniforms_offset_dev)) return BLISS_EINVAL;
  hipStream_t st = (hipStream_t)stream_;
  LayerCounts* cnt = (LayerCounts*)ws->counts;
  if (cand_bound < 1) cand_bound = 1;
  if (cand_bound > ws->cap_c) cand_bound = ws->cap_c;
  if (!ws->fs_ticket)
    PROF_LAUNCH(BK_POISSON_SCALE, st, k_poisson_scale<<<1, 1024, 0, st>>>(ws->hist, cnt, fanout, eps, rng_ctl, uniforms_offset_dev, is_last, rng_cap_total, ws->chunk_cnt));
  PROF_LAUNCH(BK_SELECT2, st, k_select_fused<<<grid_for(cand_bound, CHUNK, 1 << 20), TPB, 0, st>>>(
      (const bf16_t*)ws->p, uniforms, uniforms_offset_dev, cnt, (bf16_t*)ws->P, ws->chunk_cnt, ws->cand_nid, ws->new_id, ws->kept_nid,
      (bf16_t*)ws->node_prob, ws->cap_c, ws->cap_k, ws->kept_map));
  return (int)hipGetLastError();
}

int bliss_poisson_select_keyed(const bliss_layer_ws_t* ws, int32_t fanout, double eps, uint64_t seed, int64_t* step_dev,
                               int32_t layer, int bump_step, int64_t cand_bound, void* stream_) {
  if (!ws || !step_dev || fanout < 0 || layer < 0 || layer > 255) return BLISS_EINVAL;
  hipStream_t st = (hipStream_t)stream_;
  LayerCounts* cnt = (LayerCounts*)ws->counts;
  if (cand_bound < 1) cand_bound = 1;
  if (cand_bound > ws->cap_c) cand_bound = ws->cap_c;
  if (!ws->fs_ticket)
    PROF_LAUNCH(BK_POISSON_SCALE, st, k_poisson_scale<<<1, 1024, 0, st>>>(ws->hist, cnt, fanout, eps, nullptr, nullptr, 0, 0, ws->chunk_cnt));
  PROF_LAUNCH(BK_SELECT2, st, k_select_keyed<<<grid_for(cand_bound, CHUNK, 1 << 20), TPB, 0, st>>>(
      (const bf16_t*)ws->p, KeyedDraw{(unsigned long long)seed, (long long*)step_dev, (int)layer, bump_step ? 1 : 0}, cnt, (bf16_t*)ws->P,
      ws->chunk_cnt, ws->cand_nid, ws->new_id, ws->kept_nid, (bf16_t*)ws->node_prob, ws->cap_c, ws->cap_k, ws->kept_map));
  return (int)hipGetLastError();
}

int bliss_poisson_scale(int32_t* hist, void* counts, int32_t fanout, double eps, int32_t* scratch, void* stream_) {
  if (!hist || !counts || !scratch || fanout < 0) return BLISS_EINVAL;
  hipStream_t st = (hipStream_t)stream_;
  PROF_LAUNCH(BK_POISSON_SCALE, st, k_poisson_scale<<<1, 1024, 0, st>>>(hist, (LayerCounts*)counts, fanout, eps, nullptr, nullptr, 0, 0, scratch));
  return (int)hipGetLastError();
}

int bliss_multinomial_select(const bliss_layer_ws_t* ws, const int32_t* chosen, int32_t n_chosen, void* stream_) {
  if (!ws || n_chosen < 0 || (n_chosen > 0 && !chosen)) return BLISS_EINVAL;
  hipStream_t st = (hipStream_t)stream_;
  LayerCounts* cnt = (LayerCounts*)ws->counts;
  const int gc = grid_for(ws->cap_c, CHUNK), ge = grid_for(ws->cap_c, TPB);
  k_mn_prepare<<<ge, TPB, 0, st>>>(cnt, (const bf16_t*)ws->p, (bf16_t*)ws->P, ws->new_id, ws->cap_c);
  if (n_chosen > 0) k_mn_mark<<<grid_for(n_chosen, TPB), TPB, 0, st>>>(cnt, chosen, n_chosen, ws->new_id, ws->cap_c);
// ... 68 lines not shown
```

bliss_gnn_amd/nn.py:

```python
import torch
import torch.nn as nn

from . import _lib
from ._engine import _stream, spmm_partials


def embed_norm(h):
    from . import ops
    h = h.detach()
    if h.dtype != torch.bfloat16:
        h = h.bfloat16()
    if h.stride(1) != 1:
        h = h.contiguous()
    return ops.embed_norm(h)


def _wait_block(block):
    r = getattr(block, "_ready", None)
    if r is not None:
        _lib.check(_lib.lib.bliss_flag_wait(r[0], r[1], _stream()), "bliss_flag_wait")
        block._ready = None


def weighted_aggregate(block, h, edge_weight=None, mean=True, out_fp32=False):
    from . import ops
    assert h.is_cuda and h.dtype == torch.bfloat16, "bf16 features on the GPU (load_graph.py:7)"
    _wait_block(block)
    if h.stride(1) != 1:
        h = h.contiguous()
    w = None
    if edge_weight is not None:
        w = edge_weight.reshape(-1)
        if w.dtype != torch.bfloat16:
            w = w.bfloat16()
        w = w.contiguous()
        assert w.numel() == block.num_edges()
    counts = getattr(block, "_counts_dev", None) if block._nnz_ptr else None
    need_t = h.requires_grad and torch.is_grad_enabled()
    t_indptr, t_edge = block.transposed() if need_t else (None, None)
    return ops.spmm(block.indptr, block.src, block.dst, w, h, block.num_dst_nodes(), counts, bool(mean), bool(out_fp32), t_indptr, t_edge)


class _SageEpilogue(torch.autograd.Function):

    @staticmethod
    def forward(ctx, a, b, p, ctr, seed):
        ctx.set_materialize_grads(False)
        a, b = a.contiguous(), b.contiguous()
        n, d = a.shape
        out = torch.empty_like(a)
        norm = torch.empty(n, dtype=torch.bfloat16, device=a.device)
        _lib.check(_lib.lib.bliss_sage_epilogue_fwd(a.data_ptr(), a.stride(0), b.data_ptr(), b.stride(0), n, d, float(p), int(seed),
                                                    0 if ctr is None else ctr.data_ptr(), out.data_ptr(), out.stride(0),
                                                    norm.data_ptr(), _stream()), "bliss_sage_epilogue_fwd")
        ctx.save_for_backward(out)
        ctx.p = float(p)
        ctx.mark_non_differentiable(norm)
        return out, norm

    @staticmethod
    def backward(ctx, dout, _dnorm):
        (out,) = ctx.saved_tensors
        if dout is None:
            return None, None, None, None, None
        dout = dout.contiguous()
        if dout.dtype != torch.bfloat16:
            dout = dout.bfloat16()
        din = torch.empty_like(out)
        _lib.check(_lib.lib.bliss_sage_epilogue_bwd(dout.data_ptr(), dout.stride(0), out.data_ptr(), out.stride(0), out.shape[0],
                                                    out.shape[1], ctx.p, din.data_ptr(), din.stride(0), _stream()),
                   "bliss_sage_epilogue_bwd")
        return din, din, None, None, None


def sage_epilogue(self_out, neigh, p, ctr, seed):
    return _SageEpilogue.apply(self_out, neigh, p, ctr, seed)


_row_ids = {}


def _identity_ids(n, device):
# ... 216 lines not shown
              and a.numel() > 0 and a.stride(1) == 1 and b.stride(1) == 1 and b.device == a.device
              and label_table.dtype == torch.float32 and label_table.dim() == 2 and label_table.shape[1] == a.shape[1]
              and label_table.is_contiguous() and label_table.device == a.device and not label_table.requires_grad
              and label_ids.dtype == torch.int32 and label_ids.is_contiguous() and label_ids.numel() == a.shape[0]
              and label_ids.device == a.device)
        if not ok:
            return self.backward_from(a + b, torch.index_select(label_table, 0, label_ids.long()), n_rows_dev)
        if n_rows_dev is not None:
            n_rows_dev = _live_word(n_rows_dev, a.device)
        loss, dx = _bce_launch(a.detach(), label_table, self._state_on(a.device), x2=b.detach(), label_ids=label_ids, **_live_kw(n_rows_dev))
        torch.autograd.backward([a, b], [dx, dx])
        return loss


TILE_GEMM_MAX_K, TILE_GEMM_MAX_N = 1024, 256


class LazyRows:

    def __init__(self, table, ids, frame=None, key=None):
        self.table, self.ids, self._frame, self._key = table, ids, frame, key
        self.shape, self.dtype, self.device = (ids.numel(), table.shape[1]), table.dtype, table.device
        self.is_cuda = table.is_cuda

    def materialize(self):
        if self._frame is not None:
            return self._frame[self._key]
        return torch.index_select(self.table, 0, self.ids)


def _tg_args(a1, w1, out, m_bound, ids=None, a2=None, w2=None, bias=None, m_dev=0, a_copy=None, in_norm=None, out_norm=None,
             relu=False, p=0.0, seed=0, ctr=None):
    import ctypes as C
    t = _lib.TileGemm()
    t.a1, t.a1_stride, t.ids = a1.data_ptr(), a1.stride(0), 0 if ids is None else ids.data_ptr()
    t.w1, t.w1_stride, t.k1 = w1.data_ptr(), w1.stride(0), w1.shape[1]
    if a2 is not None:
        t.a2, t.a2_stride, t.w2, t.w2_stride, t.k2 = a2.data_ptr(), a2.stride(0), w2.data_ptr(), w2.stride(0), w2.shape[1]
    t.bias = 0 if bias is None else bias.data_ptr()
    t.m_bound, t.m_dev, t.n = int(m_bound), int(m_dev), w1.shape[0]
    t.out, t.out_stride = out.data_ptr(), out.stride(0)
    if a_copy is not None:
        t.a_copy, t.copy_stride = a_copy.data_ptr(), a_copy.stride(0)
    t.in_norm = 0 if in_norm is None else in_norm.data_ptr()
    t.out_norm = 0 if out_norm is None else out_norm.data_ptr()
    t.relu, t.drop_p, t.drop_seed, t.drop_ctr = int(relu), float(p), int(seed) & 0xFFFFFFFF, 0 if ctr is None else ctr.data_ptr()
    return t


def _tile_gemm(first, second=None):
    import ctypes as C
    _lib.check(_lib.lib.bliss_tile_gemm(C.byref(first), None if second is None else C.byref(second), _stream()), "bliss_tile_gemm")


def _bf16c(t):
    t = t if t.dtype == torch.bfloat16 else t.bfloat16()
    return t if t.stride(-1) == 1 else t.contiguous()



def _mfma_bwd_on():
    import os
    return os.environ.get("BLISS_SAGE_MFMA_BWD", "1") != "0"


def _bwd_ok(*mats):
    return all(m is None or (m.is_cuda and m.dtype == torch.bfloat16 and m.dim() == 2 and m.stride(1) == 1) for m in mats)


def sage_dgrad(a1, w1, m_bound, m_dev=0, a2=None, w2=None, m2_bound=0, m2_dev=0):
    import ctypes as C
    out = torch.empty(m_bound, w1.shape[1], dtype=torch.bfloat16, device=a1.device)
    t = _lib.DGrad()
    t.a1, t.a1_stride, t.w1, t.w1_stride, t.k1 = a1.data_ptr(), a1.stride(0), w1.data_ptr(), w1.stride(0), w1.shape[0]
    if a2 is not None:
        t.a2, t.a2_stride, t.w2, t.w2_stride, t.k2 = a2.data_ptr(), a2.stride(0), w2.data_ptr(), w2.stride(0), w2.shape[0]
        t.m2_bound, t.m2_dev = int(m2_bound), int(m2_dev)
    t.m_bound, t.m_dev, t.n = int(m_bound), int(m_dev), w1.shape[1]
    t.out, t.out_stride = out.data_ptr(), out.stride(0)
    _lib.check(_lib.lib.bliss_sage_dgrad(C.byref(t), _stream()), "bliss_sage_dgrad")
    return out


def sage_wgrad(problems):
    import ctypes as C
    n = len(problems)
    arr = (_lib.WGrad * n)()
    outs = []
    for i, (d, x, rb, rdev, want_b) in enumerate(problems):
        dw = torch.empty(d.shape[1], x.shape[1], dtype=torch.bfloat16, device=d.device)
        db = torch.empty(d.shape[1], dtype=torch.bfloat16, device=d.device) if want_b else None
        a = arr[i]
        a.d, a.d_stride, a.n_out = d.data_ptr(), d.stride(0), d.shape[1]
        a.x, a.x_stride, a.k_in = x.data_ptr(), x.stride(0), x.shape[1]
        a.rows_bound, a.rows_dev = int(rb), int(rdev)
        a.dw, a.dw_stride, a.db = dw.data_ptr(), dw.stride(0), 0 if db is None else db.data_ptr()
        outs.append((dw, db))
    need = int(_lib.lib.bliss_sage_wgrad_workspace(arr, n))
    if need < 0:
        raise RuntimeError("bliss_sage_wgrad: invalid problem description")
    ws = torch.empty(max(need, 4), dtype=torch.float32, device=problems[0][0].device)
    _lib.check(_lib.lib.bliss_sage_wgrad(arr, n, ws.data_ptr(), ws.numel(), _stream()), "bliss_sage_wgrad")
    return outs


class _SageLinearPair(torch.autograd.Function):

    @staticmethod
    def forward(ctx, x, ids, w_neigh, w_self, b_self, n_src, n_dst, src_dev, dst_dev):
        ctx.set_materialize_grads(False)
        x, wn, ws = _bf16c(x), _bf16c(w_neigh), _bf16c(w_self)
        dev, n_out = x.device, wn.shape[0]
        z = torch.empty(n_src, n_out, dtype=torch.bfloat16, device=dev)
        y = torch.empty(n_dst, n_out, dtype=torch.bfloat16, device=dev)
        norm = torch.empty(n_src, dtype=torch.bfloat16, device=dev)
        rows = torch.empty(n_src, x.shape[1], dtype=torch.bfloat16, device=dev) if ids is not None else x
        _tile_gemm(_tg_args(x, wn, z, n_src, ids=ids, m_dev=src_dev, a_copy=rows if ids is not None else None, in_norm=norm),
                   _tg_args(x, ws, y, n_dst, ids=ids, bias=b_self, m_dev=dst_dev))
        ctx.save_for_backward(rows, wn, ws)
        ctx.gathered, ctx.n_dst, ctx.has_bias = ids is not None, n_dst, b_self is not None
        ctx.n_src, ctx.src_dev, ctx.dst_dev = n_src, src_dev, dst_dev
        ctx.mark_non_differentiable(rows, norm) if ids is not None else ctx.mark_non_differentiable(norm)
        return z, y, rows, norm

    @staticmethod
    def backward(ctx, dz, dy, _drows, _dnorm):
        rows, wn, ws = ctx.saved_tensors
        want_dx = not ctx.gathered and ctx.needs_input_grad[0]
        d_wn = d_ws = d_b = dx = None
        if (_mfma_bwd_on() and dz is not None and dy is not None and wn.shape[0] <= 256 and _bwd_ok(rows, wn, ws)
                and dz.dtype == torch.bfloat16 and dy.dtype == torch.bfloat16):
            dz, dy = _bf16c(dz), _bf16c(dy)
            (d_wn, _), (d_ws, d_b) = sage_wgrad([(dz, rows, ctx.n_src, ctx.src_dev, False), (dy, rows, ctx.n_dst, ctx.dst_dev, ctx.has_bias)])
            if want_dx:
                dx = sage_dgrad(dz, wn, ctx.n_src, ctx.src_dev, a2=dy, w2=ws, m2_bound=ctx.n_dst, m2_dev=ctx.dst_dev)
                if _drows is not None:
                    dx = dx + _drows
            return dx, None, d_wn, d_ws, d_b, None, None, None, None
        if dz is not None:
            dz = _bf16c(dz)
            d_wn = _weight_grad(dz, rows)
            if want_dx:
                dx = dz @ wn
        if dy is not None:
            dy = _bf16c(dy)
            d_ws = _weight_grad(dy, rows[: ctx.n_dst])
            d_b = _bias_grad(dy) if ctx.has_bias else None
            if want_dx:
                if dx is None:
                    dx = torch.zeros_like(rows)
                dx[: ctx.n_dst].addmm_(dy, ws)
        if _drows is not None and want_dx:
            dx = _drows if dx is None else dx + _drows
        return dx, None, d_wn, d_ws, d_b, None, None, None, None


class _SageLinearSplit(torch.autograd.Function):

    @staticmethod
    def forward(ctx, x_src, x_dst, w_neigh, w_self, b_self, src_dev, dst_dev, dst_ids=None):
        ctx.set_materialize_grads(False)
        xs, wn, ws = _bf16c(x_src), _bf16c(w_neigh), _bf16c(w_self)
        dev, n_out = xs.device, wn.shape[0]
        gathered = x_dst is None
        n_dst = dst_ids.numel() if gathered else x_dst.shape[0]
        xd = torch.empty(n_dst, xs.shape[1], dtype=torch.bfloat16, device=dev) if gathered else _bf16c(x_dst)
        z = torch.empty(xs.shape[0], n_out, dtype=torch.bfloat16, device=dev)
        y = torch.empty(n_dst, n_out, dtype=torch.bfloat16, device=dev)
        norm = torch.empty(xs.shape[0], dtype=torch.bfloat16, device=dev)
        second = (_tg_args(xs, ws, y, n_dst, ids=dst_ids, bias=b_self, m_dev=dst_dev, a_copy=xd) if gathered
                  else _tg_args(xd, ws, y, n_dst, bias=b_self, m_dev=dst_dev))
        _tile_gemm(_tg_args(xs, wn, z, xs.shape[0], m_dev=src_dev, in_norm=norm), second)
        ctx.save_for_backward(xs, xd, wn, ws, dst_ids if gathered else None)
        ctx.has_bias, ctx.src_dev, ctx.dst_dev, ctx.gathered = b_self is not None, src_dev, dst_dev, gathered
        ctx.mark_non_differentiable(norm)
        return z, y, norm

    @staticmethod
    def backward(ctx, dz, dy, _dnorm):
        xs, xd, wn, ws, ids = ctx.saved_tensors
        d_wn = d_ws = d_b = dxs = dxd = None
        probs = []
        if dz is not None:
            dz = _bf16c(dz)
            probs.append((dz, xs, xs.shape[0], ctx.src_dev, False))
        if dy is not None:
            dy = _bf16c(dy)
            probs.append((dy, xd, xd.shape[0], ctx.dst_dev, ctx.has_bias))
        if probs:
            outs = sage_wgrad(probs)
            if dz is not None:
                d_wn = outs[0][0]
            if dy is not None:
                d_ws, d_b = outs[-1]
        if dz is not None and ctx.needs_input_grad[0]:
            dxs = sage_dgrad(dz, wn, xs.shape[0], ctx.src_dev)
        if dy is not None and ctx.needs_input_grad[0 if ctx.gathered else 1]:
            dxd = sage_dgrad(dy, ws, xd.shape[0], ctx.dst_dev)
            if ctx.gathered:
                dxs = torch.empty_like(xs).fill_(0) if dxs is None else dxs
                dxs.index_add_(0, ids, dxd)
                dxd = None
        return dxs, dxd, d_wn, d_ws, d_b, None, None, None


_ones_rows = {}


def _bias_grad(d):
    if not (d.is_cuda and d.dim() == 2 and d.shape[0] >= 1024):
        return d.sum(0)
    key = (d.device.index, d.dtype)
    buf = _ones_rows.get(key)
    if buf is None or buf.shape[1] < d.shape[0]:
        buf = _ones_rows[key] = torch.ones(1, max(d.shape[0], 16384), dtype=d.dtype, device=d.device)
    return (buf[:, : d.shape[0]] @ d)[0]


def _weight_grad(d, x, split=4):
    R = d.shape[0]
    if R < 8192 or x.shape[1] < 512 or R % split or not d.is_cuda:
        return d.t() @ x
    p = torch.bmm(d.view(split, R // split, d.shape[1]).transpose(1, 2), x.reshape(split, R // split, x.shape[1]), out_dtype=torch.float32)
    return p.sum(0).to(d.dtype)


class _SageDualLinear(torch.autograd.Function):

    @staticmethod
    def forward(ctx, a_neigh, a_self, w_neigh, w_self, bias, relu, p, ctr, seed, n_rows, rows_dev):
        ctx.set_materialize_grads(False)
        a1, a2, w1, w2 = _bf16c(a_neigh), _bf16c(a_self), _bf16c(w_neigh), _bf16c(w_self)
        out = torch.empty(n_rows, w1.shape[0], dtype=torch.bfloat16, device=a1.device)
        norm = torch.empty(n_rows, dtype=torch.bfloat16, device=a1.device)
        _tile_gemm(_tg_args(a1, w1, out, n_rows, a2=a2, w2=w2, bias=bias, m_dev=rows_dev, out_norm=norm, relu=relu, p=p, seed=seed, ctr=ctr))
        ctx.save_for_backward(a1, a2, w1, w2, out)
        ctx.relu, ctx.p, ctx.has_bias, ctx.rows_dev = relu, float(p), bias is not None, rows_dev
        ctx.mark_non_differentiable(norm)
        return out, norm

    @staticmethod
    def backward(ctx, dout, _dnorm):
        a1, a2, w1, w2, out = ctx.saved_tensors
        if dout is None:
            return (None,) * 11
        d = _bf16c(dout)
        if ctx.relu or ctx.p > 0:
            din = torch.empty_like(out)
            _lib.check(_lib.lib.bliss_sage_epilogue_bwd(d.data_ptr(), d.stride(0), out.data_ptr(), out.stride(0), out.shape[0],
                                                        out.shape[1], ctx.p, din.data_ptr(), din.stride(0), _stream()),
                       "bliss_sage_epilogue_bwd")
            d = din
        if _mfma_bwd_on() and w1.shape[0] <= 256 and _bwd_ok(d, a1, a2, w1, w2) and a1.shape[0] == d.shape[0] and a2.shape[0] >= d.shape[0]:
            rd = ctx.rows_dev
            (dw1, _), (dw2, db) = sage_wgrad([(d, a1, d.shape[0], rd, False), (d, a2, d.shape[0], rd, ctx.has_bias)])
            da1 = sage_dgrad(d, w1, d.shape[0], rd) if ctx.needs_input_grad[0] else None
            da2 = None
            if ctx.needs_input_grad[1]:
                da2 = sage_dgrad(d, w2, d.shape[0], rd)
                if a2.shape[0] > d.shape[0]:
                    da2 = torch.cat([da2, torch.zeros(a2.shape[0] - d.shape[0], da2.shape[1], dtype=da2.dtype, device=da2.device)])
            return (da1, da2, dw1, dw2, db, None, None, None, None, None, None)
        return (d @ w1, d @ w2, d.t() @ a1, d.t() @ a2, _bias_grad(d) if ctx.has_bias else None, None, None, None, None, None, None)


class _SageAggDual(torch.autograd.Function):

    @staticmethod
    def forward(ctx, h, indptr, src, dst, w, counts, t_indptr, t_edge, n_dst, w_neigh, w_self, bias, relu, p, ctr, seed, rows_dev):
        from . import ops
        ctx.set_materialize_grads(False)
        h, w1, w2 = _bf16c(h), _bf16c(w_neigh), _bf16c(w_self)
        agg = ops.spmm(indptr, src, dst, w, h, n_dst, counts, True, False, None, None)
        out = torch.empty(n_dst, w1.shape[0], dtype=torch.bfloat16, device=h.device)
        norm = torch.empty(n_dst, dtype=torch.bfloat16, device=h.device)
        _tile_gemm(_tg_args(agg, w1, out, n_dst, a2=h, w2=w2, bias=bias, m_dev=rows_dev, out_norm=norm, relu=relu, p=p, seed=seed, ctr=ctr))
        ctx.save_for_backward(agg, h, w1, w2, out, indptr, src, dst, w, counts, t_indptr, t_edge)
        ctx.relu, ctx.p, ctx.has_bias, ctx.n_dst, ctx.rows_dev = relu, float(p), bias is not None, n_dst, rows_dev
        ctx.mark_non_differentiable(norm)
        return out, norm

    @staticmethod
    def backward(ctx, dout, _dnorm):
        from . import ops
        agg, h, w1, w2, out, indptr, src, dst, w, counts, t_indptr, t_edge = ctx.saved_tensors
        if dout is None:
            return (None,) * 17
        d = _bf16c(dout)
        if ctx.relu or ctx.p > 0:
            din = torch.empty_like(out)
            _lib.check(_lib.lib.bliss_sage_epilogue_bwd(d.data_ptr(), d.stride(0), out.data_ptr(), out.stride(0), out.shape[0],
                                                        out.shape[1], ctx.p, din.data_ptr(), din.stride(0), _stream()),
                       "bliss_sage_epilogue_bwd")
            d = din
        gh = None
        mfma = _mfma_bwd_on() and w1.shape[0] <= 256 and _bwd_ok(d, agg, h, w1, w2)
        if ctx.needs_input_grad[0]:
            if t_indptr is None or t_edge is None:
                raise RuntimeError("the block's by-source index (Block.transposed()) is needed to differentiate w.r.t. h")
            if mfma:
                t = ops.spmm_t(t_indptr, t_edge, src, dst, indptr, w, d, h.shape[0], counts, True)
                src_dev = counts.data_ptr() + 12 if counts is not None else 0
                gh = sage_dgrad(t, w1, h.shape[0], src_dev, a2=d, w2=w2, m2_bound=ctx.n_dst, m2_dev=ctx.rows_dev)
            else:
                gh = ops.spmm_t(t_indptr, t_edge, src, dst, indptr, w, d @ w1, h.shape[0], counts, True)
                gh[: ctx.n_dst].addmm_(d, w2)
        if mfma:
            (dw1, _), (dw2, db) = sage_wgrad([(d, agg, ctx.n_dst, ctx.rows_dev, False), (d, h, ctx.n_dst, ctx.rows_dev, ctx.has_bias)])
            return (gh, None, None, None, None, None, None, None, None, dw1, dw2, db, None, None, None, None, None)
        return (gh, None, None, None, None, None, None, None, None, d.t() @ agg, d.t() @ h[: ctx.n_dst],
                _bias_grad(d) if ctx.has_bias else None, None, None, None, None, None)


def sage_agg_dual(block, h, edge_weight, w_neigh, w_self, bias, relu, p, ctr, seed, rows_dev):
    assert h.is_cuda and h.dtype == torch.bfloat16
    _wait_block(block)
    w = None
    if edge_weight is not None:
        w = edge_weight.reshape(-1)
        w = (w if w.dtype == torch.bfloat16 else w.bfloat16()).contiguous()
    counts = getattr(block, "_counts_dev", None) if block._nnz_ptr else None
    need_t = h.requires_grad and torch.is_grad_enabled()
    t_indptr, t_edge = block.transposed() if need_t else (None, None)
    return _SageAggDual.apply(h, block.indptr, block.src, block.dst, w, counts, t_indptr, t_edge, block.num_dst_nodes(), w_neigh, w_self,
                              bias, relu, p, ctr, seed, rows_dev)


def tile_gemm_ok(in_feats, out_feats):
    return in_feats <= TILE_GEMM_MAX_K and out_feats <= TILE_GEMM_MAX_N


class SAGEConv(nn.Module):

    def __init__(self, in_feats, out_feats, aggregator_type="mean", feat_drop=0.0, bias=True, norm=None, activation=None):
        super().__init__()
        if aggregator_type != "mean":
            raise NotImplementedError("the reference only builds SAGEConv(..., 'mean') (model.py:303-308)")
        self._in_src_feats = self._in_dst_feats = in_feats
        self._out_feats = out_feats
        self.feat_drop = nn.Dropout(feat_drop)
        self.norm, self.activation = norm, activation
        self.fc_neigh = nn.Linear(in_feats, out_feats, bias=False)
        self.fc_self = nn.Linear(in_feats, out_feats, bias=bias)
        self.reset_parameters()

    def reset_parameters(self):
        gain = nn.init.calculate_gain("relu")
        nn.init.xavier_uniform_(self.fc_self.weight, gain=gain)
        nn.init.xavier_uniform_(self.fc_neigh.weight, gain=gain)

    def forward(self, graph, feat, edge_weight=None, parts=False):
        if isinstance(feat, tuple):
            feat_src, feat_dst = self.feat_drop(feat[0]), self.feat_drop(feat[1])
        else:
            feat_src = self.feat_drop(feat)
            feat_dst = feat_src[: graph.num_dst_nodes()]
        lin_before_mp = self._in_src_feats > self._out_feats
        if lin_before_mp:
            h_neigh = weighted_aggregate(graph, self.fc_neigh(feat_src), edge_weight, mean=True)
        else:
            h_neigh = self.fc_neigh(weighted_aggregate(graph, feat_src, edge_weight, mean=True))
        if parts and self.activation is None and self.norm is None:
            return self.fc_self(feat_dst), h_neigh
        rst = self.fc_self(feat_dst) + h_neigh
        if self.activation is not None:
            rst = self.activation(rst)
        if self.norm is not None:
            rst = self.norm(rst)
        return rst


GCN_TRANSFORMS = ("library", "tile")


def _is_relu(act):
    return act in (torch.relu, torch.nn.functional.relu) or isinstance(act, nn.ReLU)


def _gcn_spmm(backward, idx, w, ns, nd, h, n_rows, nnz_dev):
    indptr, src, dst, t_indptr, t_edge = idx
    B, D = int(src.numel()), h.shape[1]
    out = torch.empty(n_rows, D, dtype=torch.bfloat16, device=h.device)
    part = spmm_partials(B, D, h.device, floor=4)
    wp = 0 if w is None else w.data_ptr()
    if backward:
        _lib.check(_lib.lib.bliss_gcn_spmm_bwd(t_indptr.data_ptr(), t_edge.data_ptr(), src.data_ptr(), dst.data_ptr(), wp, ns.data_ptr(),
                                               nd.data_ptr(), h.data_ptr(), h.stride(0), n_rows, nnz_dev, B, D, out.data_ptr(), out.stride(0),
                                               part.data_ptr(), _stream()), "bliss_gcn_spmm_bwd")
    else:
        _lib.check(_lib.lib.bliss_gcn_spmm_fwd(indptr.data_ptr(), src.data_ptr(), dst.data_ptr(), wp, ns.data_ptr(), nd.data_ptr(),
                                               h.data_ptr(), h.stride(0), n_rows, nnz_dev, B, D, out.data_ptr(), out.stride(0),
# ... 895 lines not shown
```

bliss_gnn_amd/train.py:

```python
import contextlib
import ctypes as C
import os
import time

import torch
import torch.nn as nn

from . import _lib


class BatchLoader:

    def __init__(self, ids, batch_size, shuffle=True, drop_last=True, seed=2):
        self.ids, self.bs, self.shuffle, self.drop_last = ids, int(batch_size), shuffle, drop_last
        self._next_bs = None
        self.gen = torch.Generator(device=ids.device)
        self.gen.manual_seed(seed)

    def set_batch_size(self, bs):
        bs = int(bs)
        if bs < 1:
            raise ValueError("batch size must be at least 1, got %d" % bs)
        self._next_bs = bs

    def __len__(self):
        n = self.ids.numel()
        return n // self.bs if self.drop_last else (n + self.bs - 1) // self.bs

    def __iter__(self):
        if self._next_bs is not None:
            self.bs, self._next_bs = self._next_bs, None
        return self._batches(self.bs, len(self))

    def _batches(self, bs, count):
        ids = self.ids
        if self.shuffle:
            ids = ids[torch.randperm(ids.numel(), generator=self.gen, device=ids.device)]
        for i in range(count):
            yield ids[i * bs:(i + 1) * bs]

    def forever(self):
        while True:
            yield from iter(self)


def _cap_kw():
    try:
        import torch.distributed as _d
        return {"capture_error_mode": "thread_local"} if _d.is_available() and _d.is_initialized() else {}
    except Exception:
        return {}


def _inputs(model, mfgs):
    if getattr(model, "accepts_lazy_rows", False):
        return mfgs[0].srcdata.lazy("features")
    return mfgs[0].srcdata["features"]


def _ce_loss():
    if os.environ.get("BLISS_FUSED_CE", "1") == "0":
        return nn.CrossEntropyLoss()
    from .nn import CrossEntropyLoss
    return CrossEntropyLoss()


def _bce_loss():
    if os.environ.get("BLISS_FUSED_BCE", "1") == "0":
        return nn.BCEWithLogitsLoss()
    from .nn import BCEWithLogitsLoss
    return BCEWithLogitsLoss()


def _loss_backward(loss_fn, pred, labels, opt, n_rows_dev=None):
    opt.zero_grad(set_to_none=True)
    if n_rows_dev is not None:
        if not hasattr(loss_fn, "backward_from"):
            raise NotImplementedError("a batch capacity needs the one-launch losses of csrc/loss.hip (BLISS_FUSED_CE / "
                                      "BLISS_FUSED_BCE are off): torch's losses have no live row count")
        return loss_fn.backward_from(pred, labels, n_rows_dev=n_rows_dev)
    if hasattr(loss_fn, "backward_from"):
        return loss_fn.backward_from(pred, labels)
    loss = loss_fn(pred, labels)
    loss.backward()
    return loss.detach()


def _update_metric(metric, pred, mfgs, n_rows_dev=None):
    lab = mfgs[-1].dstdata
    parent = getattr(lab, "_parent", None)
    if parent is not None and "labels" in parent:
        from .graph import NID
        metric.update(pred, label_table=parent["labels"], label_ids=lab[NID], n_rows_dev=n_rows_dev)
    else:
        metric.update(pred, lab["labels"], n_rows_dev=n_rows_dev)


def _live_refusal(model):
    from .model import GATv2, GCN, SAGE
    from .nn import _mfma_bwd_on
    if isinstance(model, GCN):
        if model.transforms != "tile":
            return ('GCN runs live on its bounded kernels only: with transforms="library" its layers run over all capacity rows of '
                    'the output block; build it with GCN(..., transforms="tile") (DESIGN.md section 26)')
        return model.tile_refusal()
    if isinstance(model, GATv2):
        if model.transforms != "tile":
            return ('GATv2 runs live on its bounded kernels only: with transforms="library" its layers run over all capacity rows of '
                    'the output block; build it with GATv2(..., transforms="tile") (DESIGN.md section 22)')
        ps = list(model.parameters())
        if not ps or not all(p.is_cuda and p.dtype == torch.bfloat16 for p in ps):
            return 'GATv2(transforms="tile") takes bf16 parameters on the GPU'
        return model.tile_refusal()
    if not isinstance(model, SAGE):
        return ("%s has no live path: its layers run over all capacity rows of the output block (only SAGE on its MFMA path, "
                'GATv2(transforms="tile") and GCN(transforms="tile") bound every row loop by the block\'s device-side counts)' % type(model).__name__)
    ps = list(model.parameters())
    if not ps or not model._mfma_ok(ps[0]) or not _mfma_bwd_on():
        return ("SAGE runs live on its MFMA path only (bf16 on the GPU, ReLU, layers within the tile kernel's limits, "
                "BLISS_SAGE_MFMA / BLISS_SAGE_MFMA_BWD not 0): the library-GEMM path multiplies stale capacity rows into the "
                "weight gradients")
    return None


def _check_capacity(batch_size, batch_capacity, model, what):
    cap = int(batch_capacity)
    if cap < int(batch_size) or int(batch_size) < 1:
        raise ValueError("%s: batch_capacity (%d) must be at least the batch size (%d)" % (what, cap, int(batch_size)))
    why = _live_refusal(model)
    if why is not None:
        raise NotImplementedError("%s(batch_capacity=...): %s" % (what, why))
    return cap


def _train_metric(train_metric, multilabel):
    if not train_metric:
        return None
    from .metrics import MicroF1
    return MicroF1(multilabel)


def make_adam(model, lr, capturable=False):
    ps = list(model.parameters())
    if ps and all(p.is_cuda and p.dtype == torch.bfloat16 and p.is_contiguous() for p in ps) and len(ps) <= _lib.ADAM_MAX_TENSORS:
        from .optim import Adam
        return Adam(ps, lr=lr)
    if capturable:
        return torch.optim.Adam(ps, lr=lr, capturable=True, fused=True)
    return torch.optim.Adam(ps, lr=lr)


class TrainStep:

    def __init__(self, g, sampler, model, lr=0.002, multilabel=False, bandit=True, grad_sync=None, exp3_sync=None, train_metric=False):
        self.g, self.sampler, self.model = g, sampler, model
        self.loss_fn = _bce_loss() if multilabel else _ce_loss()
        self.train_acc = _train_metric(train_metric, multilabel)
        self.opt = make_adam(model, lr)
        self.bandit = bandit and hasattr(sampler, "exp3")
        self.grad_sync, self.exp3_sync = grad_sync, exp3_sync
        self.num_steps = 0
        self.w = 0.99
        n_layers = len(sampler.nodes_per_layer)
        self.cum_sampled_nodes = [0.0] * (n_layers + 1)
        self.cum_sampled_edges = [0.0] * n_layers
        self.last = {}

    def _ema(self, mfgs):
# ... 394 lines not shown

    def close(self):
        import gc
        torch.cuda.synchronize()
        for name in self._graph_attrs():
            v = getattr(self, name, None)
            if isinstance(v, list):
                setattr(self, name, [None] * len(v))
            elif v is not None:
                setattr(self, name, None)
        self.loss = None
        if hasattr(self, "losses"):
            self.losses = None
        gc.collect()
        torch.cuda.synchronize()


class PipelinedTrainStep(GraphedTrainStep):

    def __init__(self, g, sampler, model, batch_size, lr=0.002, multilabel=False, distributed=False, train_metric=False,
                 batch_capacity=None):
        if batch_capacity is not None:
            raise NotImplementedError("PipelinedTrainStep has no batch_capacity: its sampler is split over streams around a "
                                      "host-known seed count (use GraphedTrainStep)")
        if train_metric:
            raise NotImplementedError("PipelinedTrainStep keeps no train_acc (its forward pass is split over two graphs and two "
                                      "streams): use TrainStep or GraphedTrainStep with train_metric=True")
        if getattr(sampler, "draw", "host") == "device":
            raise NotImplementedError("PipelinedTrainStep splits the sampler over streams and runs its generator beside it; the "
                                      "device-side draws (multinomial, neighbor) have neither: use GraphedTrainStep with draw='device'")
        super().__init__(g, sampler, model, batch_size, lr, multilabel, distributed)
        self.seeds2 = [torch.zeros(self.bs, dtype=torch.int32, device=g.device) for _ in range(2)]
        self.mfgs = [None, None]
        self.side = torch.cuda.Stream()
        self.third = torch.cuda.Stream()
        self._fwd_done, self._bwd_done, self._blk_done = torch.cuda.Event(), torch.cuda.Event(), torch.cuda.Event()
        self._seed_ev = torch.cuda.Event()
        self.use_flags = os.environ.get("BLISS_PIPELINE_FLAGS", "1") != "0"
        self.losses = None
        self.last_counts2 = None
        self._flag_boundary = os.environ.get("BLISS_FLAG_BOUNDARY", "1") != "0"
        self._defer_block0 = False
        self.g_blk0 = [None, None]
        self._blk0_done = torch.cuda.Event()

    def _sample(self, slot, chain, external_rng=False, part=None, last_block=True, ready_flag=0):
        return self.sampler.sample_blocks_static(self.g, self.seeds2[slot], slot=slot, chain_rng=chain, external_rng=external_rng,
                                                 part=part, last_block=last_block, ready_flag=ready_flag)[2]

    def _split_forward(self):
        return (hasattr(self.model, "forward_hidden") and len(getattr(self.model, "layers", ())) > 1 and hasattr(self.sampler, "exp3")
                and os.environ.get("BLISS_SPLIT_FORWARD", "1") != "0")

    FLAG_BLOCK0, FLAG_B_DONE = 10, 11

    def _forward(self, mfgs):
        pending = self._forward_model(mfgs)
        if not hasattr(self.sampler, "exp3"):
            return pending
        if self.distributed:
            from . import dist as bdist
            bdist.exp3_all_ranks_static(self.sampler, mfgs, self.g)
        else:
            self.sampler.exp3(mfgs, self.g)
        return pending

    def _forward_model(self, mfgs):
        if self._split_forward():
            pending = ("hidden", self.model.forward_hidden(mfgs, _inputs(self.model, mfgs)), mfgs)
        else:
            pred = self.model(mfgs, _inputs(self.model, mfgs))
            pending = ("pred", pred, mfgs)
        return pending

    def _backward(self, pending):
        kind, val, mfgs = pending
        loss = None
        if kind == "hidden" and hasattr(self.model, "forward_last_parts") and hasattr(self.loss_fn, "backward_from_parts"):
            lab = mfgs[-1].dstdata
            table = lab._parent["labels"] if getattr(lab, "_parent", None) is not None and "labels" in lab._parent else None
            parts = self.model.forward_last_parts(mfgs, val) if table is not None and not dict.__contains__(lab, "labels") else None
            if parts is not None:
                self.opt.zero_grad(set_to_none=True)
                loss = self.loss_fn.backward_from_parts(parts[0], parts[1], table, lab._index_fn())
        if loss is None:
            pred = self.model.forward_last(mfgs, val) if kind == "hidden" else val
            loss = _loss_backward(self.loss_fn, pred, mfgs[-1].dstdata["labels"], self.opt)
        if self.distributed:
            from . import dist as bdist
            bdist.allreduce_gradients(self.model)
        self.opt.step()
        return loss

    def _pair(self):
        main, side = torch.cuda.current_stream(), self.side
        side.wait_stream(main)
        losses = []
        for cur, nxt, chain in ((0, 1, False), (1, 0, True)):
            with torch.cuda.stream(side):
                pending = self._forward(self.mfgs[cur])
            main.wait_stream(side)
            self.mfgs[nxt] = self._sample(nxt, chain)
            with torch.cuda.stream(side):
                losses.append(self._backward(pending))
                side.wait_stream(main)
        main.wait_stream(side)
        return tuple(losses)

    def prime(self, seeds):
        self.seeds2[0].copy_(seeds)
        self.sampler._engine.stage_rng_from_torch()
        self.mfgs[0] = self._sample(0, False)
        torch.cuda.current_stream().synchronize()
        self.sampler.finish_static(0, commit=True)

    def _finish_pair(self, check_flags=True):
        torch.cuda.current_stream().synchronize()
        c1 = self.sampler.finish_static(1, commit=False)
        c0 = self.sampler.finish_static(0, commit=True)
        self.last_counts2 = [c1, c0]
        self.last_counts = c0
        self.num_steps += 2
        if check_flags and self.graph and self.use_flags and int(self.sampler._engine.flag_err.item()):
            raise RuntimeError("a cross-stream flag never arrived (bliss_flag_wait timed out): the pipelined results are invalid")

    def _load(self, loader):
        self.seeds2[1].copy_(next(loader))
        self.seeds2[0].copy_(next(loader))
        self.sampler._engine.stage_rng_from_torch()

    def capture(self, loader, warmup=2, tune_gemm=False):
        eng = self.sampler._bind(self.g)
        L = len(self.sampler.nodes_per_layer)
        if torch.cuda.current_stream() != torch.cuda.default_stream():
            import warnings
            warnings.warn("PipelinedTrainStep: captured from a non-default stream; HIP maps streams onto a few hardware queues and the "
                          "critical chain then shares one with a side stream (measured 1.08 instead of 0.70 ms per step)")
        if self.use_flags and not self._flags_usable():
            import warnings
            warnings.warn("PipelinedTrainStep: streams do not run side by side here (a profiler serialising kernels?); "
                          "ordering the graphs with events instead of device flags")
            self.use_flags = False
        if self.use_flags:
            eng.scratch_sets = max(eng.scratch_sets, L)
        self._defer_block0 = (self.use_flags and self._flag_boundary and L > 1 and L < self.FLAG_BLOCK0 and type(self.model).__name__ == "SAGE"
                              and self._split_forward() and os.environ.get("BLISS_DEFER_BLOCK0", "1") != "0")
        tune_gemm = tune_gemm and _enable_gemm_tuning()
        warm = torch.cuda.Stream()
        warm.wait_stream(torch.cuda.current_stream())
        with torch.cuda.stream(warm):
            self.prime(next(loader))
            for _ in range(warmup):
                self._load(loader)
                self.losses = self._pair()
                self._finish_pair()
        torch.cuda.current_stream().wait_stream(warm)
        if tune_gemm:
            torch.cuda.tunable.tuning_enable(False)
        self.losses = None
        import gc
        gc.collect()
        torch.cuda.synchronize()
        self._capture_graphs(loader)
        if self.use_flags and int(eng.flag_err.item()):
            import warnings
            warnings.warn("PipelinedTrainStep: a cross-stream flag timed out (streams sharing a hardware queue?); "
                          "falling back to event-ordered graphs")
# ... 572 lines not shown
```

include/bliss_gnn.h:

```cpp
#ifndef BLISS_GNN_H
#define BLISS_GNN_H
#include <stdint.h>

#ifdef __cplusplus
extern "C" {
#endif

#define BLISS_EINVAL (-1)

#define BLISS_MODE_BANDIT 0
#define BLISS_MODE_LADIES 1
#define BLISS_ROWSUM_SLOTS 32
#define BLISS_NORM_SCRATCH (2 + 3 * BLISS_ROWSUM_SLOTS)
#define BLISS_MODE_UNIFORM_NODES 4
#define BLISS_MODE_PARTIALS 8

typedef struct {
  const int64_t* indptr;
  const int32_t* indices;
  const int32_t* eid;
  int32_t num_nodes;
  int64_t num_edges;
} bliss_graph_t;

// ... 117 lines not shown
int bliss_labor_is_layer(const bliss_graph_t* g, const int32_t* seeds, int32_t n_seeds, const int32_t* n_seeds_dev, int32_t cap_s,
                         int32_t fanout, const uint32_t* keys_override, uint64_t seed, int64_t* step_dev, int32_t layer,
                         int bump_step, int layer_dependency, int32_t iterations, const bliss_layer_ws_t* ws,
                         const bliss_block_out_t* out, void* scratch, void* stream);

int64_t bliss_wlabor_scratch_bytes(int32_t num_nodes, int32_t cap_s, int32_t cap_b);
int bliss_wlabor_layer(const bliss_graph_t* g, const int32_t* seeds, int32_t n_seeds, const int32_t* n_seeds_dev, int32_t cap_s,
                       int32_t fanout, const uint32_t* keys_override, uint64_t seed, int64_t* step_dev, int32_t layer, int bump_step,
                       int layer_dependency, int32_t mode, const void* prob_pos, float eta, float one_minus_eta,
                       const bliss_layer_ws_t* ws, const bliss_block_out_t* out, void* p_ij, void* scratch, void* stream);

int bliss_build_block(const bliss_graph_t* g, const bliss_node_maps_t* maps, const void* w_pos,
                      const int32_t* seeds, int32_t cap_s, int mode, float eta_f, float one_minus_eta_f,
                      int64_t frontier_bound, const bliss_layer_ws_t* ws, const bliss_block_out_t* out, void* stream);

int bliss_mt19937_uniform(void* state, const int32_t* n_dev, int32_t n_word_offset, float* out, int32_t cap, void* stream);

int bliss_rng_stream_begin(const void* state, int32_t* ctl, float* out, uint32_t* raw, int32_t cap_total, void* stream);
int bliss_rng_prepare(int32_t cap_total, int32_t* plan4);
int bliss_mt_jump_poly(int64_t n_words, uint32_t* poly_words);
int bliss_rng_stream_wait(int32_t* ctl, const void* counts, int32_t* layer_off, int is_last, int32_t cap_total, void* stream);
int bliss_rng_stream_end(void* state, const int32_t* ctl, const uint32_t* raw, int32_t cap_total, int32_t* err_word,
                         void* stream);
int bliss_rng_stream_chain(void* state, int32_t* ctl, float* out, uint32_t* raw, int32_t cap_total, int32_t* counts_dev,
                           int32_t n_count_words, int32_t* counts_host, void* stream);
int bliss_rng_stream_ready(void* stream);
int64_t bliss_rng_stream_handle(void);

int bliss_cand_importance(const int64_t* sums, int32_t n, int uniform_nodes, void* p_bf16, int32_t* err, void* stream);
int bliss_poisson_scale(int32_t* hist, void* counts, int32_t fanout, double eps, int32_t* scratch, void* stream);
int bliss_keyed_select(const int32_t* nid, const void* p_bf16, const uint8_t* is_seed, int32_t n, const void* counts,
                       uint64_t seed, uint64_t step, int32_t layer, void* P_bf16, uint8_t* keep, void* stream);
int bliss_shard_local_seeds(const int32_t* seeds_g, int32_t n_seeds, const int32_t* n_seeds_dev, int32_t lo, int32_t hi, int32_t cap_s,
                            int32_t* seeds_l, int32_t* seeds_l_copy, int32_t* seed_pos, int32_t* n_local_dev, int32_t* err, void* stream);
int bliss_shard_scatter_partials(const int32_t* seeds_l, const int64_t* seed_p2, const int32_t* n_local_dev, const int64_t* touched_key,
                                 const int64_t* touched_sum, const int32_t* n_touched_dev, int64_t* dense, int32_t num_nodes,
                                 int32_t* err, void* stream);
int bliss_shard_pack_rows(const int32_t* nid, const int32_t* n_rows_dev, int32_t cap_rows, int32_t lo, int32_t hi, const void* table_bf16,
                          int64_t table_stride, int32_t row_len, void* out_bf16, int64_t out_stride, void* stream);
int bliss_shard_place_rows(const void* src_bf16, int64_t src_stride, const int32_t* pos, const int32_t* n_dev, int32_t cap_s, void* out_bf16,
                           int64_t out_stride, int32_t n_rows, int32_t row_len, void* stream);
int bliss_shard_take_rows(const void* src, int32_t src_is_f32, int64_t src_stride, int32_t n_src_rows, const int32_t* pos, const int32_t* n_dev,
                          int32_t cap_s, void* out_bf16, int64_t out_stride, int32_t row_len, void* stream);
int bliss_shard_zero_dense(int64_t* dense, int32_t num_nodes, void* stream);
int bliss_shard_candidates(int64_t* dense, int32_t num_nodes, int32_t uniform_nodes, int32_t* cand_nid, void* p_bf16, uint8_t* is_seed,
                           int32_t* hist, void* counts, int32_t cap_c, int32_t* scratch, int32_t* err, void* stream);
int bliss_shard_select_kept(const int32_t* cand_nid, const void* p_bf16, const uint8_t* is_seed, const void* counts, uint64_t seed,
                            int64_t* step_dev, int32_t layer, const int32_t* seeds_g, int32_t n_seeds, const int32_t* n_seeds_dev,
                            void* P_bf16, int32_t* kept_nid, void* node_prob_bf16, int32_t* kept_map, int32_t cap_k, int32_t cap_c,
                            int32_t num_nodes, void* layer_counts, const int32_t* n_local_dev, int32_t* scratch, int32_t bump_step,
                            int32_t* done_flag, int32_t* err, void* stream);
int bliss_exp3_normalize_global(void* w_pos, int64_t num_edges, int64_t* row_sum, const int64_t* norm_limbs, int64_t* scratch,
                                void* norm_out_bf16, void* stream);

typedef struct {
  const void* a1; int64_t a1_stride; const int32_t* ids;
  const void* w1; int64_t w1_stride; int32_t k1;
  const void* a2; int64_t a2_stride; const void* w2; int64_t w2_stride; int32_t k2;
  const void* bias;
  int32_t m_bound; const int32_t* m_dev; int32_t n;
  void* out; int64_t out_stride;
  void* a_copy; int64_t copy_stride;
  void* in_norm; void* out_norm;
  int32_t relu; float drop_p; uint32_t drop_seed; void* drop_ctr;
} bliss_tile_gemm_t;
int bliss_tile_gemm(const bliss_tile_gemm_t* first, const bliss_tile_gemm_t* second_or_null, void* stream);

typedef struct {
  const void* a1; int64_t a1_stride; const void* w1; int64_t w1_stride; int32_t k1;
  const void* a2; int64_t a2_stride; const void* w2; int64_t w2_stride; int32_t k2; int32_t m2_bound; const int32_t* m2_dev;
  int32_t m_bound; const int32_t* m_dev; int32_t n;
  void* out; int64_t out_stride;
} bliss_dgrad_t;
int bliss_sage_dgrad(const bliss_dgrad_t* args, void* stream);
int bliss_gat_dgrad(const bliss_dgrad_t* args, void* stream);
typedef struct {
  const void* d; int64_t d_stride; int32_t n_out;
  const void* x; int64_t x_stride; int32_t k_in;
  int32_t rows_bound; const int32_t* rows_dev;
  void* dw; int64_t dw_stride; void* db;
} bliss_wgrad_t;
int64_t bliss_sage_wgrad_workspace(const bliss_wgrad_t* probs, int32_t n_probs);
int bliss_sage_wgrad(const bliss_wgrad_t* probs, int32_t n_probs, float* partials, int64_t partial_floats, void* stream);

int bliss_cross_entropy(const void* logits, int64_t stride, const int64_t* labels, int32_t n_rows, int32_t n_cls,
                        float* row_loss, void* dlogits, int64_t d_stride, float* loss_out, uint32_t* ticket, int32_t* err,
                        void* stream);
int bliss_cross_entropy_sum(const void* logits, int64_t stride, const void* logits2, int64_t stride2, const int64_t* label_table,
                            const int32_t* label_ids, int32_t n_rows, int32_t n_cls, float* row_loss, void* dlogits, int64_t d_stride,
                            float* loss_out, uint32_t* ticket, int32_t* err, void* stream);
int bliss_cross_entropy_masked(const void* logits, int64_t stride, const void* logits2, int64_t stride2, const int64_t* label_table,
                               int32_t n_table, const int32_t* label_ids, int32_t id_off, int32_t n_rows, const int32_t* n_rows_dev,
                               float denom, int32_t n_cls, float* row_loss, void* dlogits, int64_t d_stride, float* loss_out,
                               uint32_t* ticket, int32_t* err, void* stream);

int bliss_cross_entropy_live(const void* logits, int64_t stride, const void* logits2, int64_t stride2, const int64_t* label_table,
                             const int32_t* label_ids, int32_t n_rows, const int32_t* n_rows_dev, int32_t n_cls, float* row_loss,
                             void* dlogits, int64_t d_stride, float* loss_out, uint32_t* ticket, int32_t* err, void* stream);

int bliss_bce_logits(const void* logits, int64_t stride, const float* targets, int32_t n_rows, int32_t n_cls, float* row_loss,
                     void* dlogits, int64_t d_stride, float* loss_out, uint32_t* ticket, int32_t* err, void* stream);
int bliss_bce_logits_sum(const void* logits, int64_t stride, const void* logits2, int64_t stride2, const float* target_table,
                         const int32_t* label_ids, int32_t n_rows, int32_t n_cls, float* row_loss, void* dlogits, int64_t d_stride,
                         float* loss_out, uint32_t* ticket, int32_t* err, void* stream);
int bliss_bce_logits_masked(const void* logits, int64_t stride, const void* logits2, int64_t stride2, const float* target_table,
                            int32_t n_table, const int32_t* label_ids, int32_t id_off, int32_t n_rows, const int32_t* n_rows_dev,
                            float denom, int32_t n_cls, float* row_loss, void* dlogits, int64_t d_stride, float* loss_out,
                            uint32_t* ticket, int32_t* err, void* stream);

int bliss_bce_logits_live(const void* logits, int64_t stride, const void* logits2, int64_t stride2, const float* target_table,
                          const int32_t* label_ids, int32_t n_rows, const int32_t* n_rows_dev, int32_t n_cls, float* row_loss,
                          void* dlogits, int64_t d_stride, float* loss_out, uint32_t* ticket, int32_t* err, void* stream);

#define BLISS_F1_MAX_WORKGROUPS 1024
int bliss_f1_multiclass(const void* logits, int64_t stride, int32_t n_pred_rows, const int32_t* row_ids, const int64_t* labels,
                        const int64_t* label_table, int32_t n_table, const int32_t* label_ids, int32_t n_rows,
                        const int32_t* n_rows_dev, int32_t n_cls, int64_t* counts, int32_t* err, void* stream);
int bliss_f1_multilabel(const void* logits, int64_t stride, int32_t n_pred_rows, const int32_t* row_ids, const float* labels,
                        const float* label_table, int32_t n_table, const int32_t* label_ids, int32_t n_rows,
                        const int32_t* n_rows_dev, int32_t n_cls, int64_t* counts, int32_t* err, void* stream);

#define BLISS_ADAM_MAX_TENSORS 32
typedef struct {
  void* param[BLISS_ADAM_MAX_TENSORS];
  const void* grad[BLISS_ADAM_MAX_TENSORS];
  void* exp_avg[BLISS_ADAM_MAX_TENSORS];
  void* exp_avg_sq[BLISS_ADAM_MAX_TENSORS];
  int64_t numel[BLISS_ADAM_MAX_TENSORS];
  int32_t count;
} bliss_adam_t;
int bliss_adam_step(const bliss_adam_t* tensors, float* state, float beta1, float beta2, float eps, float weight_decay, void* stream);

#define BLISS_LEDGER_MAX_LAYERS 8
#define BLISS_LEDGER_STEP 0
#define BLISS_LEDGER_RESET_EPOCH 1
#define BLISS_LEDGER_REARM 2
#define BLISS_LEDGER_LOSS_BF16 0
#define BLISS_LEDGER_LOSS_F32 1
int bliss_step_ledger_bytes(int n_layers);
int bliss_step_ledger(int mode, const void* loss, int loss_dtype, const int32_t* counts, int n_layers, const int32_t* caps,
                      double w, double regrow_at, void* ledger, void* stream);

#define BLISS_BATCH_STATS_BYTES 32
#define BLISS_BATCH_STATS_PUSH 0
#define BLISS_BATCH_STATS_CLEAR 1
int bliss_batch_stats(int mode, const int32_t* counts, int layer, void* record, void* stream);

int bliss_normalized_edata(const bliss_graph_t* g, void* w_pos, void* stream);

int bliss_gather_rows(const void* feat, int64_t feat_stride, const int32_t* ids, int32_t n_rows, int32_t dim, void* out,
                      int64_t out_stride, void* norm_out, void* stream);

int bliss_embed_norm(const void* h, int32_t n_rows, int32_t dim, int64_t row_stride, void* out, void* stream);

int bliss_spmm_chunk_edges(int32_t nnz_bound);
int bliss_spmm_fwd(const int32_t* indptr, const int32_t* src, const int32_t* dst, const void* w, const void* h,
                   int64_t h_stride, int32_t n_dst, const int32_t* nnz_dev, int32_t nnz, int32_t dim, int mean, void* out,
                   int64_t out_stride, int out_fp32, float* partials, void* stream);

int bliss_spmm_bwd(const int32_t* t_indptr, const int32_t* t_edge, const int32_t* src, const int32_t* dst,
                   const int32_t* indptr, const void* w, const void* gout, int64_t gout_stride, int32_t n_src,
                   const int32_t* nnz_dev, int32_t nnz, int32_t dim, int mean, void* gh, int64_t gh_stride, int out_fp32,
                   float* partials, void* stream);

int bliss_sage_epilogue_fwd(const void* a, int64_t a_stride, const void* b, int64_t b_stride, int32_t n_rows, int32_t dim,
                            float p_drop, uint32_t seed, uint64_t* ctr, void* out, int64_t out_stride, void* norm_out, void* stream);
// ... 167 lines not shown
```

Baseline: 1555.

## Batch SAGE weight-gradient launches across layers and split seed scan into front kernel

During backward, SAGE weight-gradient problems are no longer launched one node at a time. They are deferred and then launched together through a new batched wgrad entry point, which packs up to three problem groups into one wgrad kernel and one reduce kernel, ordered by workgroup count. Separately, the sampler's segment scan is split: a parallel front kernel reads seed degrees and builds the long-column list, and a leaner scan follows; the seed accumulator buffer grows and is now zero-initialised. The goal is fewer kernel launches and better GPU occupancy. The cost is deferred gradient bookkeeping and a larger launch struct.

Result: no change. 1568, median of 6 (+0.9%).

```diff
diff --git a/bliss_gnn_amd/_engine.py b/bliss_gnn_amd/_engine.py
--- a/bliss_gnn_amd/_engine.py
+++ b/bliss_gnn_amd/_engine.py
@@ -158,7 +158,7 @@
     def __init__(self, dev, cap_s, cap_c):
         self.cap_s, self.cap_c = cap_s, cap_c
         self.seg_ptr = torch.empty(cap_s + 1, dtype=torch.int32, device=dev)
-        self.seed_acc = torch.empty(72 * cap_s + 64, dtype=torch.uint8, device=dev)
+        self.seed_acc = torch.zeros(88 * cap_s + 64, dtype=torch.uint8, device=dev)
         self.cand_nid = torch.empty(cap_c, dtype=torch.int32, device=dev)
         self.new_id = torch.empty(cap_c, dtype=torch.int32, device=dev)
         self.p = torch.empty(cap_c, dtype=torch.bfloat16, device=dev)
diff --git a/bliss_gnn_amd/_lib.py b/bliss_gnn_amd/_lib.py
--- a/bliss_gnn_amd/_lib.py
+++ b/bliss_gnn_amd/_lib.py
@@ -284,6 +284,7 @@
     "bliss_gat_logits": [_P, _P, _P, _I32, _P, _I64, _P, _I32, _I32, _F, _P, _P],
     "bliss_sage_dgrad": [C.POINTER(DGrad), _P],
     "bliss_sage_wgrad": [C.POINTER(WGrad), _I32, _P, _I64, _P],
+    "bliss_sage_wgrad_batch": [C.POINTER(WGrad), C.POINTER(C.c_int32), _I32, _P, _I64, _P],
     "bliss_gat_dgrad": [C.POINTER(DGrad), _P],
     "bliss_gat_glue_fwd": [C.POINTER(GatGlue), _P],
     "bliss_gat_glue_bwd": [C.POINTER(GatGlue), _P],
@@ -327,6 +328,7 @@
 
 SPECIAL_SIGNATURES = ("bliss_prof_kernel_name", "bliss_block_transpose_temp_bytes", "bliss_graph_prepare_capacity",
                       "bliss_graph_prepare_temp_bytes", "bliss_rng_stream_handle", "bliss_sage_wgrad_workspace",
+                      "bliss_sage_wgrad_batch_workspace",
                       "bliss_multinomial_draw_scratch_bytes", "bliss_neighbor_scratch_bytes", "bliss_wneighbor_scratch_bytes",
                       "bliss_labor_scratch_bytes", "bliss_labor_is_scratch_bytes", "bliss_wlabor_scratch_bytes",
                       "bliss_neighbor_replace_scratch_bytes", "bliss_multinomial_draw_replace_scratch_bytes")
@@ -346,6 +348,8 @@
     lib.bliss_block_transpose_temp_bytes.restype = C.c_int64
     lib.bliss_sage_wgrad_workspace.argtypes = [C.POINTER(WGrad), _I32]
     lib.bliss_sage_wgrad_workspace.restype = C.c_int64
+    lib.bliss_sage_wgrad_batch_workspace.argtypes = [C.POINTER(WGrad), C.POINTER(C.c_int32), _I32]
+    lib.bliss_sage_wgrad_batch_workspace.restype = C.c_int64
     for name in ("bliss_graph_prepare_capacity", "bliss_graph_prepare_temp_bytes"):
         getattr(lib, name).argtypes = [_I64, _I32, C.c_int]
         getattr(lib, name).restype = C.c_int64
diff --git a/bliss_gnn_amd/csrc/sage_bwd.hip b/bliss_gnn_amd/csrc/sage_bwd.hip
--- a/bliss_gnn_amd/csrc/sage_bwd.hip
+++ b/bliss_gnn_amd/csrc/sage_bwd.hip
@@ -147,6 +147,7 @@
 #define WG_DSTRIDE (256 + 32)
 #define WG_XSTRIDE (WG_TN + 32)
 #define WG_MAX_PROBS 2
+#define WG_MAX_LAUNCH 6
 
 struct WGradProb {
   const bf16_t* d; long long d_stride; int n_out;
@@ -157,7 +158,7 @@
   int ldp;
   int wg_begin;
 };
-struct WGradLaunch { WGradProb p[WG_MAX_PROBS]; int n; };
+struct WGradLaunch { WGradProb p[WG_MAX_LAUNCH]; int n; };
 
 struct WRegsB { uint4 d[2]; uint4 x; };
 
@@ -185,7 +186,8 @@
   __shared__ __attribute__((aligned(16))) bf16_t dimg[WG_ROWS * WG_DSTRIDE];
   __shared__ __attribute__((aligned(16))) bf16_t ximg[WG_ROWS * WG_XSTRIDE];
   const int tid = threadIdx.x, wave = tid >> 6, lane = tid & 63;
-  const int pi = (L.n > 1 && (int)blockIdx.x >= L.p[1].wg_begin) ? 1 : 0;
+  int pi = 0;
+  for (int i = 1; i < L.n; ++i) if ((int)blockIdx.x >= L.p[i].wg_begin) pi = i;
   const WGradProb& p = L.p[pi];
   const int w = (int)blockIdx.x - p.wg_begin;
   const int ct = w % p.col_tiles, ch = w / p.col_tiles;
@@ -320,6 +322,49 @@
   return true;
 }
 
+bool wgrad_plan_groups(const bliss_wgrad_t* a, const int32_t* group_sizes, int n_groups, WGradLaunch* L, long long* floats,
+                       int* total_wgs) {
+  if (!a || !group_sizes || n_groups < 1 || n_groups * WG_MAX_PROBS > WG_MAX_LAUNCH) return false;
+  WGradLaunch G[WG_MAX_LAUNCH / WG_MAX_PROBS];
+  long long g_floats[WG_MAX_LAUNCH / WG_MAX_PROBS];
+  int g_wgs[WG_MAX_LAUNCH / WG_MAX_PROBS], order[WG_MAX_LAUNCH / WG_MAX_PROBS];
+  for (int g = 0, at = 0; g < n_groups; at += group_sizes[g], ++g) {
+    if (group_sizes[g] < 1 || group_sizes[g] > WG_MAX_PROBS || !wgrad_plan(a + at, group_sizes[g], &G[g], &g_floats[g], &g_wgs[g])) return false;
+    int i = g;
+    for (; i > 0 && g_wgs[order[i - 1]] < g_wgs[g]; --i) order[i] = order[i - 1];
+    order[i] = g;
+  }
+  long long off = 0;
+  int wgs = 0, n = 0;
+  for (int o = 0; o < n_groups; ++o) {
+    const int g = order[o];
+    for (int i = 0; i < G[g].n; ++i) {
+      WGradProb& p = L->p[n++];
+      p = G[g].p[i];
+      p.part_off += off;
+      p.wg_begin += wgs;
+    }
+    off += g_floats[g];
+    wgs += g_wgs[g];
+  }
+  L->n = n;
+  *floats = off;
+  *total_wgs = wgs;
+  return true;
+}
+
+int wgrad_launch(const WGradLaunch& L, int wgs, long long floats, float* partials, int64_t partial_floats, void* stream) {
+  if (partial_floats < floats || (((uintptr_t)partials) % 16) != 0) return BLISS_EINVAL;
+  hipStream_t st = (hipStream_t)stream;
+  k_wgrad<<<wgs, WG_TPB, 0, st>>>(L, partials);
+  int max_elems = 0;
+  for (int i = 0; i < L.n; ++i) { const int e = L.p[i].n_out * ((L.p[i].k_in + 3) / 4 + 1); if (e > max_elems) max_elems = e; }
+  int gx = (max_elems + 255) / 256;
+  if (gx > 1024) gx = 1024;
+  k_wgrad_reduce<<<dim3(gx, L.n), 256, 0, st>>>(L, partials);
+  return (int)hipGetLastError();
+}
+
 int dgrad_launch(const bliss_dgrad_t* a, int k_max, void* stream) {
   if (!a || !a->a1 || !a->w1 || !a->out || a->k1 <= 0 || a->k1 > k_max || a->n <= 0 || a->m_bound <= 0) return BLISS_EINVAL;
   if (a->k2 < 0 || a->k2 > k_max || (a->k2 > 0 && (!a->a2 || !a->w2 || a->m2_bound <= 0))) return BLISS_EINVAL;
@@ -364,15 +409,24 @@
   long long floats = 0;
   int wgs = 0;
   if (!probs || !partials || !wgrad_plan(probs, n_probs, &L, &floats, &wgs)) return BLISS_EINVAL;
-  if (partial_floats < floats || (((uintptr_t)partials) % 16) != 0) return BLISS_EINVAL;
-  hipStream_t st = (hipStream_t)stream;
-  k_wgrad<<<wgs, WG_TPB, 0, st>>>(L, partials);
-  int max_elems = 0;
-  for (int i = 0; i < n_probs; ++i) { const int e = L.p[i].n_out * ((L.p[i].k_in + 3) / 4 + 1); if (e > max_elems) max_elems = e; }
-  int gx = (max_elems + 255) / 256;
-  if (gx > 1024) gx = 1024;
-  k_wgrad_reduce<<<dim3(gx, n_probs), 256, 0, st>>>(L, partials);
-  return (int)hipGetLastError();
-}
-
-}
+  return wgrad_launch(L, wgs, floats, partials, partial_floats, stream);
+}
+
+int64_t bliss_sage_wgrad_batch_workspace(const bliss_wgrad_t* probs, const int32_t* group_sizes, int32_t n_groups) {
+  WGradLaunch L;
+  long long floats = 0;
+  int wgs = 0;
+  if (!wgrad_plan_groups(probs, group_sizes, n_groups, &L, &floats, &wgs)) return -1;
+  return (int64_t)floats;
+}
+
+int bliss_sage_wgrad_batch(const bliss_wgrad_t* probs, const int32_t* group_sizes, int32_t n_groups, float* partials,
+                           int64_t partial_floats, void* stream) {
+  WGradLaunch L;
+  long long floats = 0;
+  int wgs = 0;
+  if (!partials || !wgrad_plan_groups(probs, group_sizes, n_groups, &L, &floats, &wgs)) return BLISS_EINVAL;
+  return wgrad_launch(L, wgs, floats, partials, partial_floats, stream);
+}
+
+}
diff --git a/bliss_gnn_amd/csrc/sampler.hip b/bliss_gnn_amd/csrc/sampler.hip
--- a/bliss_gnn_amd/csrc/sampler.hip
+++ b/bliss_gnn_amd/csrc/sampler.hip
@@ -76,23 +76,47 @@
   return off;
 }
 
+__device__ __forceinline__ int scan_err_bits(int bad) {
+  return (bad & ~BLISS_ERR_CAP_CAND) | (__syncthreads_or(bad & BLISS_ERR_CAP_CAND) ? BLISS_ERR_CAP_CAND : 0);
+}
+
+__device__ __forceinline__ void scan_round_tables(int k, int kbase, int S, int deg, long long col, long long run, int ex, int tot,
+                                                  int* __restrict__ seg_ptr, long long* __restrict__ col_base,
+                                                  int* __restrict__ span_seg, long long frontier_cap, int* st_sh) {
+  const long long start = run + ex;
+  if (k < S) {
+    seg_ptr[k] = (int)start;
+    col_base[k] = deg > 0 ? col - start : 0;
+  }
+  if (run + tot <= frontier_cap) {
+    st_sh[threadIdx.x] = (int)(k < S ? start : run + tot);
+    __syncthreads();
+    const long long sp_end = (run + tot + SPAN - 1) / SPAN;
+    for (long long sp = (run + SPAN - 1) / SPAN + threadIdx.x; sp < sp_end; sp += blockDim.x) {
+      const int p = (int)(sp * SPAN);
+      int t = 0;
+#pragma unroll
+      for (int step = 512; step >= 1; step >>= 1) if (st_sh[t + step] <= p) t += step;
+      span_seg[sp] = kbase + t;
+    }
+  }
+}
+
 __device__ __forceinline__ void seg_scan_body(const int64_t* __restrict__ indptr, const int* __restrict__ seeds,
                                               LayerCounts* cnt, int S_host, const int* __restrict__ S_dev, int cap_s,
                                               unsigned long long* __restrict__ seed_acc, int* __restrict__ seg_ptr,
                                               int* __restrict__ local_id, int num_nodes, int* __restrict__ src_cnt, int cap_k,
                                               int* __restrict__ bin_cursor, int n_bins, long long* __restrict__ col_base,
                                               int* __restrict__ span_seg, long long frontier_cap, int* entry_flag,
-                                              int wg, int n_wgs, bool keep_sums, int* sh, int* st_sh, ColEnt* long_list = nullptr) {
+                                              int wg, int n_wgs, int* sh, int* st_sh) {
   if (entry_flag && wg == 0 && threadIdx.x == 0) __hip_atomic_store(entry_flag, 1, __ATOMIC_RELEASE, __HIP_MEMORY_SCOPE_AGENT);
-  __shared__ int sh_long[2];
-  if (long_list && threadIdx.x < 2) sh_long[threadIdx.x] = 0;
   int S = S_host >= 0 ? S_host : *S_dev;
   int bad = 0;
   if (S > cap_s) { S = cap_s; bad |= BLISS_ERR_CAP_SEEDS; }
   if (wg > 0 || n_wgs == 1) {
     const int nz = n_wgs > 1 ? n_wgs - 1 : 1, bz = n_wgs > 1 ? wg - 1 : 0;
     const int t0 = bz * blockDim.x + threadIdx.x, step = nz * blockDim.x;
-    for (int i = (keep_sums ? 2 * cap_s : 0) + t0; i < cap_s * 5; i += step) seed_acc[i] = 0ull;
+    for (int i = t0; i < cap_s * 5; i += step) seed_acc[i] = 0ull;
     if (src_cnt) for (int i = t0; i <= cap_k; i += step) src_cnt[i] = 0;
     if (bin_cursor) for (int i = t0; i <= n_bins; i += step) bin_cursor[i] = 0;
     for (int k = t0; k < S; k += step) { const int s = seeds[k]; if (s >= 0 && s < num_nodes) local_id[s] = k; }
@@ -122,50 +146,15 @@
       if (base0 + i * (int)blockDim.x >= S) break;
       const int deg = degs[i];
       int tot, ex = block_excl_scan(deg, sh, &tot);
-      const long long start = run + ex;
-      if (k < S) {
-        seg_ptr[k] = (int)start;
-        col_base[k] = deg > 0 ? cols[i] - start : 0;
-      }
-      if (long_list) {
-        const bool is_long = k < S && deg > LONG_COL, is_first = is_long && deg > LONG_FIRST;
-        const unsigned long long m_first = __ballot(is_first), m_rest = __ballot(is_long && !is_first);
-        if (m_first | m_rest) {
-          int b_first = 0, b_rest = 0;
-          if (lane_id() == 0) {
-            if (m_first) b_first = atomicAdd(&sh_long[0], __popcll(m_first));
-            if (m_rest) b_rest = atomicAdd(&sh_long[1], __popcll(m_rest));
-          }
-          b_first = __shfl(b_first, 0); b_rest = __shfl(b_rest, 0);
-          if (is_long) {
-            const unsigned long long below = (1ull << lane_id()) - 1ull;
-            const int slot = is_first ? b_first + __popcll(m_first & below) : cap_s - 1 - (b_rest + __popcll(m_rest & below));
-            ColEnt ent; ent.k = k; ent.n = deg; ent.p0 = cols[i];
-            long_list[slot] = ent;
-          }
-        }
-      }
-      if (run + tot <= frontier_cap) {
-        st_sh[threadIdx.x] = (int)(k < S ? start : run + tot);
-        __syncthreads();
-        const long long sp_end = (run + tot + SPAN - 1) / SPAN;
-        for (long long sp = (run + SPAN - 1) / SPAN + threadIdx.x; sp < sp_end; sp += blockDim.x) {
-          const int p = (int)(sp * SPAN);
-          int t = 0;
-#pragma unroll
-          for (int step = 512; step >= 1; step >>= 1) if (st_sh[t + step] <= p) t += step;
-          span_seg[sp] = base0 + i * (int)blockDim.x + t;
-        }
-      }
+      scan_round_tables(k, base0 + i * (int)blockDim.x, S, deg, cols[i], run, ex, tot, seg_ptr, col_base, span_seg, frontier_cap, st_sh);
       run += tot;
       if (run > frontier_cap) bad |= BLISS_ERR_CAP_FRONTIER;
     }
   }
-  int any_bad = __syncthreads_or(bad);
+  const int any_bad = scan_err_bits(bad);
   if (threadIdx.x == 0) {
-    if (long_list) { int* n_long = (int*)(long_list + cap_s); n_long[0] = sh_long[0]; n_long[1] = sh_long[1]; }
     seg_ptr[S] = (int)run;
-    cnt->S = S; cnt->E = (any_bad & BLISS_ERR_CAP_FRONTIER) ? 0 : (int)run;
+    cnt->S = S; cnt->E = any_bad ? 0 : (int)run;
     cnt->C = 0; cnt->K = 0; cnt->B = 0; cnt->iters = 0; cnt->all_one = 0; cnt->c = 1.0;
     cnt->err = any_bad;
   }
@@ -176,12 +165,106 @@
                                                    unsigned long long* __restrict__ seed_acc, int* __restrict__ seg_ptr,
                                                    int* __restrict__ local_id, int num_nodes, int* __restrict__ src_cnt, int cap_k,
                                                    int* __restrict__ bin_cursor, int n_bins, long long* __restrict__ col_base,
-                                                   int* __restrict__ span_seg, long long frontier_cap, int* entry_flag,
-                                                   int keep_sums, ColEnt* long_list) {
+                                                   int* __restrict__ span_seg, long long frontier_cap, int* entry_flag) {
   __shared__ int sh[17];
   __shared__ int st_sh[1024];
   seg_scan_body(indptr, seeds, cnt, S_host, S_dev, cap_s, seed_acc, seg_ptr, local_id, num_nodes, src_cnt, cap_k, bin_cursor, n_bins,
-                col_base, span_seg, frontier_cap, entry_flag, blockIdx.x, gridDim.x, keep_sums != 0, sh, st_sh, long_list);
+                col_base, span_seg, frontier_cap, entry_flag, blockIdx.x, gridDim.x, sh, st_sh);
+}
+
+struct alignas(16) SeedCol {
+  long long p0;
+  int n;
+  int pad;
+};
+#define FRONT_TPB 256
+
+__global__ void __launch_bounds__(FRONT_TPB) k_seed_front(const int64_t* __restrict__ indptr, const int* __restrict__ seeds,
+                                                          LayerCounts* cnt, int S_host, const int* __restrict__ S_dev, int cap_s,
+                                                          unsigned long long* __restrict__ seed_acc, int* __restrict__ local_id,
+                                                          int num_nodes, int* __restrict__ src_cnt, int cap_k,
+                                                          int* __restrict__ bin_cursor, int n_bins, int* entry_flag,
+                                                          SeedCol* __restrict__ seed_col, ColEnt* __restrict__ long_list) {
+  const int t0 = blockIdx.x * FRONT_TPB + threadIdx.x, step = gridDim.x * FRONT_TPB;
+  if (entry_flag && t0 == 0) __hip_atomic_store(entry_flag, 1, __ATOMIC_RELEASE, __HIP_MEMORY_SCOPE_AGENT);
+  int S = S_host >= 0 ? S_host : *S_dev;
+  int err0 = 0;
+  if (S > cap_s) { S = cap_s; err0 = BLISS_ERR_CAP_SEEDS; }
+  if (t0 == 0) {
+    cnt->S = S; cnt->C = 0; cnt->K = 0; cnt->B = 0; cnt->iters = 0; cnt->all_one = 0; cnt->c = 1.0;
+    cnt->err = err0;
+  }
+  for (int i = 2 * cap_s + t0; i < cap_s * 5; i += step) seed_acc[i] = 0ull;
+  if (src_cnt) for (int i = t0; i <= cap_k; i += step) src_cnt[i] = 0;
+  for (int i = t0; i <= n_bins; i += step) bin_cursor[i] = 0;
+  int* n_long = (int*)(long_list + cap_s);
+  const int lane = lane_id();
+  for (int kb = t0 - lane; kb < S; kb += step) {
+    const int k = kb + lane;
+    SeedCol c; c.p0 = 0; c.n = 0; c.pad = 0;
+    if (k < S) {
+      const int s = seeds[k];
+      if (s < 0 || s >= num_nodes) c.n = -1;
+      else {
+        c.p0 = indptr[s];
+        c.n = (int)(indptr[s + 1] - c.p0);
+        local_id[s] = k;
+      }
+      seed_col[k] = c;
+    }
+    const bool is_long = c.n > LONG_COL, is_first = c.n > LONG_FIRST;
+    const unsigned long long m_first = __ballot(is_first), m_rest = __ballot(is_long && !is_first);
+    if (m_first | m_rest) {
+      int b_first = 0, b_rest = 0;
+      if (lane == 0) {
+        if (m_first) b_first = atomicAdd(&n_long[0], __popcll(m_first));
+        if (m_rest) b_rest = atomicAdd(&n_long[1], __popcll(m_rest));
+      }
+      b_first = __shfl(b_first, 0); b_rest = __shfl(b_rest, 0);
+      if (is_long) {
+        const unsigned long long below = (1ull << lane) - 1ull;
+        const int slot = is_first ? b_first + __popcll(m_first & below) : cap_s - 1 - (b_rest + __popcll(m_rest & below));
+        ColEnt ent; ent.k = k; ent.n = c.n; ent.p0 = c.p0;
+        if (slot >= 0 && slot < cap_s) long_list[slot] = ent;
+      }
+    }
+  }
+}
+
+__device__ __forceinline__ void seed_scan_wg(const SeedCol* __restrict__ seed_col, LayerCounts* cnt, int* __restrict__ seg_ptr,
+                                          long long* __restrict__ col_base, int* __restrict__ span_seg, long long frontier_cap) {
+  __shared__ int sh[17];
+  __shared__ int st_sh[1024];
+  const int S = cnt->S;
+  int bad = 0;
+  long long run = 0;
+  constexpr int G = 4;
+  for (int base0 = 0; base0 < S; base0 += G * 1024) {
+    SeedCol c[G];
+#pragma unroll
+    for (int i = 0; i < G; ++i) {
+      const int k = base0 + i * 1024 + (int)threadIdx.x;
+      c[i].p0 = 0; c[i].n = 0;
+      if (k < S) c[i] = seed_col[k];
+    }
+#pragma unroll
+    for (int i = 0; i < G; ++i) {
+      const int kbase = base0 + i * 1024, k = kbase + (int)threadIdx.x;
+      if (kbase >= S) break;
+      int deg = c[i].n;
+      if (deg < 0) { deg = 0; bad |= BLISS_ERR_CAP_CAND; }
+      int tot, ex = block_excl_scan(deg, sh, &tot);
+      scan_round_tables(k, kbase, S, deg, c[i].p0, run, ex, tot, seg_ptr, col_base, span_seg, frontier_cap, st_sh);
+      run += tot;
+      if (run > frontier_cap) bad |= BLISS_ERR_CAP_FRONTIER;
+    }
+  }
+  const int any_bad = scan_err_bits(bad);
+  if (threadIdx.x == 0) {
+    seg_ptr[S] = (int)run;
+    cnt->E = any_bad ? 0 : (int)run;
+    if (any_bad) atomicOr(&cnt->err, any_bad);
+  }
 }
 
 template <bool BANDIT>
@@ -406,7 +489,7 @@
 #define COL_BLOCK_WGS 512
 #endif
 #define COL_BIG (COL_R * 64)
-static_assert(LONG_COL == COL_BIG, "k_seg_scan lists the columns k_col_sums treats as long");
+static_assert(LONG_COL == COL_BIG, "k_seed_front lists the columns k_col_sums treats as long");
 #ifndef BINRED_TPB
 #define BINRED_TPB 1024
 #endif
@@ -469,27 +552,28 @@
   seed_coef[k] = make_uint2((unsigned)wsum | ((unsigned)qsum << 16), __float_as_uint(rbf((1.0f / (float)n) * eta_f)));
 }
 
-__global__ void __launch_bounds__(COL_TPB, 8) k_col_sums(const int64_t* __restrict__ indptr, const bf16_t* __restrict__ w,
-                                                      const int* __restrict__ seeds, const int* __restrict__ seg_ptr,
-                                                      const long long* __restrict__ col_base, const int* __restrict__ span_seg,
+__global__ void __launch_bounds__(COL_TPB, 8) k_col_sums(const bf16_t* __restrict__ w, const SeedCol* __restrict__ seed_col,
+                                                      int* __restrict__ seg_ptr, long long* __restrict__ col_base,
+                                                      int* __restrict__ span_seg, long long frontier_cap,
                                                       LayerCounts* cnt, unsigned long long* __restrict__ acc_w,
                                                       unsigned long long* __restrict__ acc_q, float eta_f, float ome_f,
                                                       uint2* __restrict__ seed_coef, int n_block_wgs,
                                                       const ColEnt* __restrict__ long_list, int cap_s) {
   __shared__ long long sh[COL_TPB / 64];
   __shared__ long long sh2[2 * COL_TPB / 64];
+  if (blockIdx.x == 0) { seed_scan_wg(seed_col, cnt, seg_ptr, col_base, span_seg, frontier_cap); return; }
   const int tid = threadIdx.x, lane = lane_id();
   const int* n_long = (const int*)(long_list + cap_s);
-  const int S = cnt->S, E = cnt->E, n_first = n_long[0], n_all = n_first + n_long[1];
-  if (E == 0) return;
+  const int S = cnt->S, n_first = max(0, min(n_long[0], cap_s)), n_all = n_first + max(0, min(n_long[1], cap_s - n_first));
   int bad = 0;
-  const int bid_wave = (int)blockIdx.x, bid_block = (int)blockIdx.x - ((int)gridDim.x - n_block_wgs);
+  const int bid_wave = (int)blockIdx.x - 1, bid_block = (int)blockIdx.x - ((int)gridDim.x - n_block_wgs);
   if (bid_block < 0) {
   const int k = bid_wave * (COL_TPB / 64) + __builtin_amdgcn_readfirstlane(tid >> 6);
-  const int s0 = k < S ? seg_ptr[k] : 0, n = k < S ? seg_ptr[k + 1] - s0 : 0;
-  const long long cb = k < S ? col_base[k] : 0;
+  SeedCol sc; sc.p0 = 0; sc.n = 0;
+  if (k < S) sc = seed_col[k];
+  const int n = sc.n;
   if (n > 0 && n <= COL_BIG) {
-    const bf16_t* wc = uniform_ptr(w + (cb + s0));
+    const bf16_t* wc = uniform_ptr(w + sc.p0);
     PackedBf<COL_R> wr;
     long long part = 0;
     int emax = 1;
@@ -650,10 +734,11 @@
                                                      const unsigned long long* __restrict__ acc_q, float eta_f, float ome_f,
                                                      int uniform_nodes, int n_bins, int log2_bins, long long bin_cap, int* bin_cursor,
                                                      unsigned long long* __restrict__ bin_rec, unsigned* __restrict__ bitmap,
-                                                     const uint2* __restrict__ seed_coef) {
+                                                     const uint2* __restrict__ seed_coef, int* n_long_reset) {
   __shared__ int hist[MAX_BINS];
   __shared__ int gbase[MAX_BINS];
   const int S = cnt->S, E = cnt->E, tid = threadIdx.x;
+  if (n_long_reset && blockIdx.x == 0 && tid < 2) n_long_reset[tid] = 0;
   const int nb = (E + BIN_BATCH - 1) / BIN_BATCH;
   const int bmask = n_bins - 1;
   int bad = 0;
@@ -1536,10 +1621,18 @@
   const long long fcap = (long long)(g->num_edges < 0x7fffffffll ? g->num_edges : 0x7fffffffll);
   const bool col_sums = binned && mode == BLISS_MODE_BANDIT;
   ColEnt* long_list = (ColEnt*)(acc_w + 7 * (size_t)cap_s);
-  PROF_LAUNCH(BK_SEG_SCAN, st, k_seg_scan<<<1 + SEG_ZERO_WGS, 1024, 0, st>>>(g->indptr, seeds, cnt, n_seeds, n_seeds_dev, cap_s, acc_w, ws->seg_ptr,
-                                                            m->local_id, g->num_nodes, ws->src_cnt, ws->cap_k,
-                                                            binned ? ws->bin_cursor : nullptr, ws->n_bins, (long long*)col_base, ws->span_seg,
-                                                            fcap, ws->entry_flag, col_sums ? 1 : 0, col_sums ? long_list : nullptr));
+  SeedCol* seed_col = (SeedCol*)((char*)ws->seed_acc + ((72 * (size_t)cap_s + 8 + 15) & ~(size_t)15));
+  if (col_sums) {
+    const int most = cap_s > ws->cap_k ? cap_s : ws->cap_k;
+    PROF_LAUNCH(BK_SEG_SCAN, st, k_seed_front<<<grid_for(most, FRONT_TPB, 512), FRONT_TPB, 0, st>>>(
+        g->indptr, seeds, cnt, n_seeds, n_seeds_dev, cap_s, acc_w, m->local_id, g->num_nodes, ws->src_cnt, ws->cap_k, ws->bin_cursor,
+        ws->n_bins, ws->entry_flag, seed_col, long_list));
+  } else {
+    PROF_LAUNCH(BK_SEG_SCAN, st, k_seg_scan<<<1 + SEG_ZERO_WGS, 1024, 0, st>>>(g->indptr, seeds, cnt, n_seeds, n_seeds_dev, cap_s, acc_w, ws->seg_ptr,
+                                                              m->local_id, g->num_nodes, ws->src_cnt, ws->cap_k,
+                                                              binned ? ws->bin_cursor : nullptr, ws->n_bins, (long long*)col_base, ws->span_seg,
+                                                              fcap, ws->entry_flag));
+  }
   if (binned) {
     unsigned long long* seed_p2 = acc_w + 4 * (size_t)cap_s;
     uint2* seed_coef = (uint2*)(acc_w + 6 * (size_t)cap_s);
@@ -1547,11 +1640,11 @@
     const int gb = grid_for(frontier_bound, BIN_BATCH);
     const int n_wave_wgs = (cap_s + COL_TPB / 64 - 1) / (COL_TPB / 64), n_block_wgs = cap_s < COL_BLOCK_WGS ? cap_s : COL_BLOCK_WGS;
     if (col_sums)
-      PROF_LAUNCH(BK_COL_SUMS, st, k_col_sums<<<n_block_wgs + n_wave_wgs, COL_TPB, 0, st>>>(g->indptr, w, seeds, ws->seg_ptr, col_base, ws->span_seg, cnt, acc_w, acc_q, eta_f, one_minus_eta_f, seed_coef, n_block_wgs, long_list, cap_s));
+      PROF_LAUNCH(BK_COL_SUMS, st, k_col_sums<<<1 + n_wave_wgs + n_block_wgs, COL_TPB, 0, st>>>(w, seed_col, ws->seg_ptr, (long long*)col_base, ws->span_seg, fcap, cnt, acc_w, acc_q, eta_f, one_minus_eta_f, seed_coef, n_block_wgs, long_list, cap_s));
     if (mode == BLISS_MODE_BANDIT)
-      PROF_LAUNCH(BK_BIN_SCATTER, st, k_bin_scatter<true><<<gb, BIN_TPB, 0, st>>>(g->indptr, g->indices, w, seeds, ws->seg_ptr, col_base, ws->span_seg, cnt, acc_w, acc_q, eta_f, one_minus_eta_f, uniform_nodes, ws->n_bins, log2_bins, ws->bin_cap, ws->bin_cursor, bin_rec, ws->bitmap, seed_coef));
+      PROF_LAUNCH(BK_BIN_SCATTER, st, k_bin_scatter<true><<<gb, BIN_TPB, 0, st>>>(g->indptr, g->indices, w, seeds, ws->seg_ptr, col_base, ws->span_seg, cnt, acc_w, acc_q, eta_f, one_minus_eta_f, uniform_nodes, ws->n_bins, log2_bins, ws->bin_cap, ws->bin_cursor, bin_rec, ws->bitmap, seed_coef, (int*)(long_list + cap_s)));
     else
-      PROF_LAUNCH(BK_BIN_SCATTER, st, k_bin_scatter<false><<<gb, BIN_TPB, 0, st>>>(g->indptr, g->indices, w, seeds, ws->seg_ptr, col_base, ws->span_seg, cnt, acc_w, acc_q, eta_f, one_minus_eta_f, uniform_nodes, ws->n_bins, log2_bins, ws->bin_cap, ws->bin_cursor, bin_rec, ws->bitmap, seed_coef));
+      PROF_LAUNCH(BK_BIN_SCATTER, st, k_bin_scatter<false><<<gb, BIN_TPB, 0, st>>>(g->indptr, g->indices, w, seeds, ws->seg_ptr, col_base, ws->span_seg, cnt, acc_w, acc_q, eta_f, one_minus_eta_f, uniform_nodes, ws->n_bins, log2_bins, ws->bin_cap, ws->bin_cursor, bin_rec, ws->bitmap, seed_coef, nullptr));
     PROF_LAUNCH(BK_BIN_REDUCE, st, k_bin_reduce<<<ws->n_bins, BINRED_TPB, (size_t)slots * 12, st>>>(
         cnt, ws->n_bins, log2_bins, ws->bin_cap, ws->bin_cursor, bin_rec, g->num_nodes, slots, m->local_id, seed_p2,
         (unsigned long long*)ws->touched_key, (unsigned long long*)ws->touched_sum, ws->bitmap, ws->cap_c));
diff --git a/bliss_gnn_amd/nn.py b/bliss_gnn_amd/nn.py
--- a/bliss_gnn_amd/nn.py
+++ b/bliss_gnn_amd/nn.py
@@ -1,3 +1,6 @@
+import contextlib
+import os
+
 import torch
 import torch.nn as nn
 
@@ -380,26 +383,94 @@
     return out
 
 
-def sage_wgrad(problems):
-    import ctypes as C
-    n = len(problems)
-    arr = (_lib.WGrad * n)()
+def _wgrad_args(problems):
+    arr = (_lib.WGrad * len(problems))()
     outs = []
-    for i, (d, x, rb, rdev, want_b) in enumerate(problems):
+    for a, (d, x, rb, rdev, want_b) in zip(arr, problems):
         dw = torch.empty(d.shape[1], x.shape[1], dtype=torch.bfloat16, device=d.device)
         db = torch.empty(d.shape[1], dtype=torch.bfloat16, device=d.device) if want_b else None
-        a = arr[i]
         a.d, a.d_stride, a.n_out = d.data_ptr(), d.stride(0), d.shape[1]
         a.x, a.x_stride, a.k_in = x.data_ptr(), x.stride(0), x.shape[1]
         a.rows_bound, a.rows_dev = int(rb), int(rdev)
         a.dw, a.dw_stride, a.db = dw.data_ptr(), dw.stride(0), 0 if db is None else db.data_ptr()
         outs.append((dw, db))
+    return arr, outs
+
+
+def sage_wgrad_batch(groups):
+    import ctypes as C
+    flat = [p for g in groups for p in g]
+    arr, outs = _wgrad_args(flat)
+    sizes = (C.c_int32 * len(groups))(*[len(g) for g in groups])
+    need = int(_lib.lib.bliss_sage_wgrad_batch_workspace(arr, sizes, len(groups)))
+    if need < 0:
+        raise RuntimeError("bliss_sage_wgrad_batch: invalid problem description")
+    ws = torch.empty(max(need, 4), dtype=torch.float32, device=flat[0][0].device)
+    _lib.check(_lib.lib.bliss_sage_wgrad_batch(arr, sizes, len(groups), ws.data_ptr(), ws.numel(), _stream()), "bliss_sage_wgrad_batch")
+    res, at = [], 0
+    for g in groups:
+        res.append(outs[at: at + len(g)])
+        at += len(g)
+    return res
+
+
+def sage_wgrad(problems):
+    n = len(problems)
+    arr, outs = _wgrad_args(problems)
     need = int(_lib.lib.bliss_sage_wgrad_workspace(arr, n))
     if need < 0:
         raise RuntimeError("bliss_sage_wgrad: invalid problem description")
     ws = torch.empty(max(need, 4), dtype=torch.float32, device=problems[0][0].device)
     _lib.check(_lib.lib.bliss_sage_wgrad(arr, n, ws.data_ptr(), ws.numel(), _stream()), "bliss_sage_wgrad")
     return outs
+
+
+_deferred = None
+
+
+def _leaf_params(*ps):
+    for q in ps:
+        if q is not None and not (isinstance(q, torch.nn.Parameter) and q.is_leaf and q.requires_grad and q.dtype == torch.bfloat16):
+            return None
+    return ps
+
+
+def _node_params(ps):
+    return None if ps is None else [(ps[0], None), (ps[1], ps[2])]
+
+
+def _wgrad_node(problems, params):
+    if _deferred is None or params is None:
+        return sage_wgrad(problems)
+    _deferred.append((problems, params))
+    return [(None, None)] * len(problems)
+
+
+@contextlib.contextmanager
+def deferred_wgrads():
+    global _deferred
+    if _deferred is not None or os.environ.get("BLISS_WGRAD_BATCH", "1") == "0":
+        yield
+        return
+    _deferred = []
+    try:
+        yield
+        groups = _deferred
+    finally:
+        _deferred = None
+    for i in range(0, len(groups), 3):
+        batch = groups[i: i + 3]
+        outs = sage_wgrad_batch([g[0] for g in batch])
+        with torch.no_grad():
+            for (_, params), res in zip(batch, outs):
+                for (pw, pb), (dw, db) in zip(params, res):
+                    for q, gq in ((pw, dw), (pb, db)):
+                        if q is None or gq is None:
+                            continue
+                        if q.grad is None:
+                            q.grad = gq
+                        else:
+                            q.grad.add_(gq)
 
 
 class _SageLinearPair(torch.autograd.Function):
@@ -418,6 +489,7 @@
         ctx.save_for_backward(rows, wn, ws)
         ctx.gathered, ctx.n_dst, ctx.has_bias = ids is not None, n_dst, b_self is not None
         ctx.n_src, ctx.src_dev, ctx.dst_dev = n_src, src_dev, dst_dev
+        ctx.params = _leaf_params(w_neigh, w_self, b_self)
         ctx.mark_non_differentiable(rows, norm) if ids is not None else ctx.mark_non_differentiable(norm)
         return z, y, rows, norm
 
@@ -429,7 +501,8 @@
         if (_mfma_bwd_on() and dz is not None and dy is not None and wn.shape[0] <= 256 and _bwd_ok(rows, wn, ws)
                 and dz.dtype == torch.bfloat16 and dy.dtype == torch.bfloat16):
             dz, dy = _bf16c(dz), _bf16c(dy)
-            (d_wn, _), (d_ws, d_b) = sage_wgrad([(dz, rows, ctx.n_src, ctx.src_dev, False), (dy, rows, ctx.n_dst, ctx.dst_dev, ctx.has_bias)])
+            (d_wn, _), (d_ws, d_b) = _wgrad_node([(dz, rows, ctx.n_src, ctx.src_dev, False), (dy, rows, ctx.n_dst, ctx.dst_dev, ctx.has_bias)],
+                                                 _node_params(ctx.params))
             if want_dx:
                 dx = sage_dgrad(dz, wn, ctx.n_src, ctx.src_dev, a2=dy, w2=ws, m2_bound=ctx.n_dst, m2_dev=ctx.dst_dev)
                 if _drows is not None:
@@ -471,6 +544,7 @@
         _tile_gemm(_tg_args(xs, wn, z, xs.shape[0], m_dev=src_dev, in_norm=norm), second)
         ctx.save_for_backward(xs, xd, wn, ws, dst_ids if gathered else None)
         ctx.has_bias, ctx.src_dev, ctx.dst_dev, ctx.gathered = b_self is not None, src_dev, dst_dev, gathered
+        ctx.params = _leaf_params(w_neigh, w_self, b_self)
         ctx.mark_non_differentiable(norm)
         return z, y, norm
 
@@ -478,7 +552,7 @@
     def backward(ctx, dz, dy, _dnorm):
         xs, xd, wn, ws, ids = ctx.saved_tensors
         d_wn = d_ws = d_b = dxs = dxd = None
-        probs = []
+        probs, params = [], _node_params(ctx.params)
         if dz is not None:
             dz = _bf16c(dz)
             probs.append((dz, xs, xs.shape[0], ctx.src_dev, False))
@@ -486,7 +560,9 @@
             dy = _bf16c(dy)
             probs.append((dy, xd, xd.shape[0], ctx.dst_dev, ctx.has_bias))
         if probs:
-            outs = sage_wgrad(probs)
+            if params is not None and len(probs) == 1:
+                params = params[:1] if dz is not None else params[1:]
+            outs = _wgrad_node(probs, params)
             if dz is not None:
                 d_wn = outs[0][0]
             if dy is not None:
@@ -534,6 +610,7 @@
         _tile_gemm(_tg_args(a1, w1, out, n_rows, a2=a2, w2=w2, bias=bias, m_dev=rows_dev, out_norm=norm, relu=relu, p=p, seed=seed, ctr=ctr))
         ctx.save_for_backward(a1, a2, w1, w2, out)
         ctx.relu, ctx.p, ctx.has_bias, ctx.rows_dev = relu, float(p), bias is not None, rows_dev
+        ctx.params = _leaf_params(w_neigh, w_self, bias)
         ctx.mark_non_differentiable(norm)
         return out, norm
 
@@ -551,7 +628,7 @@
             d = din
         if _mfma_bwd_on() and w1.shape[0] <= 256 and _bwd_ok(d, a1, a2, w1, w2) and a1.shape[0] == d.shape[0] and a2.shape[0] >= d.shape[0]:
             rd = ctx.rows_dev
-            (dw1, _), (dw2, db) = sage_wgrad([(d, a1, d.shape[0], rd, False), (d, a2, d.shape[0], rd, ctx.has_bias)])
+            (dw1, _), (dw2, db) = _wgrad_node([(d, a1, d.shape[0], rd, False), (d, a2, d.shape[0], rd, ctx.has_bias)], _node_params(ctx.params))
             da1 = sage_dgrad(d, w1, d.shape[0], rd) if ctx.needs_input_grad[0] else None
             da2 = None
             if ctx.needs_input_grad[1]:
@@ -575,6 +652,7 @@
         _tile_gemm(_tg_args(agg, w1, out, n_dst, a2=h, w2=w2, bias=bias, m_dev=rows_dev, out_norm=norm, relu=relu, p=p, seed=seed, ctr=ctr))
         ctx.save_for_backward(agg, h, w1, w2, out, indptr, src, dst, w, counts, t_indptr, t_edge)
         ctx.relu, ctx.p, ctx.has_bias, ctx.n_dst, ctx.rows_dev = relu, float(p), bias is not None, n_dst, rows_dev
+        ctx.params = _leaf_params(w_neigh, w_self, bias)
         ctx.mark_non_differentiable(norm)
         return out, norm
 
@@ -604,7 +682,8 @@
                 gh = ops.spmm_t(t_indptr, t_edge, src, dst, indptr, w, d @ w1, h.shape[0], counts, True)
                 gh[: ctx.n_dst].addmm_(d, w2)
         if mfma:
-            (dw1, _), (dw2, db) = sage_wgrad([(d, agg, ctx.n_dst, ctx.rows_dev, False), (d, h, ctx.n_dst, ctx.rows_dev, ctx.has_bias)])
+            (dw1, _), (dw2, db) = _wgrad_node([(d, agg, ctx.n_dst, ctx.rows_dev, False), (d, h, ctx.n_dst, ctx.rows_dev, ctx.has_bias)],
+                                              _node_params(ctx.params))
             return (gh, None, None, None, None, None, None, None, None, dw1, dw2, db, None, None, None, None, None)
         return (gh, None, None, None, None, None, None, None, None, d.t() @ agg, d.t() @ h[: ctx.n_dst],
                 _bias_grad(d) if ctx.has_bias else None, None, None, None, None, None)
diff --git a/bliss_gnn_amd/train.py b/bliss_gnn_amd/train.py
--- a/bliss_gnn_amd/train.py
+++ b/bliss_gnn_amd/train.py
@@ -7,6 +7,7 @@
 import torch.nn as nn
 
 from . import _lib
+from .nn import deferred_wgrads
 
 
 class BatchLoader:
@@ -74,16 +75,17 @@
 
 def _loss_backward(loss_fn, pred, labels, opt, n_rows_dev=None):
     opt.zero_grad(set_to_none=True)
-    if n_rows_dev is not None:
-        if not hasattr(loss_fn, "backward_from"):
-            raise NotImplementedError("a batch capacity needs the one-launch losses of csrc/loss.hip (BLISS_FUSED_CE / "
-                                      "BLISS_FUSED_BCE are off): torch's losses have no live row count")
-        return loss_fn.backward_from(pred, labels, n_rows_dev=n_rows_dev)
-    if hasattr(loss_fn, "backward_from"):
-        return loss_fn.backward_from(pred, labels)
-    loss = loss_fn(pred, labels)
-    loss.backward()
-    return loss.detach()
+    if n_rows_dev is not None and not hasattr(loss_fn, "backward_from"):
+        raise NotImplementedError("a batch capacity needs the one-launch losses of csrc/loss.hip (BLISS_FUSED_CE / "
+                                  "BLISS_FUSED_BCE are off): torch's losses have no live row count")
+    with deferred_wgrads():
+        if n_rows_dev is not None:
+            return loss_fn.backward_from(pred, labels, n_rows_dev=n_rows_dev)
+        if hasattr(loss_fn, "backward_from"):
+            return loss_fn.backward_from(pred, labels)
+        loss = loss_fn(pred, labels)
+        loss.backward()
+        return loss.detach()
 
 
 def _update_metric(metric, pred, mfgs, n_rows_dev=None):
@@ -644,7 +646,8 @@
             parts = self.model.forward_last_parts(mfgs, val) if table is not None and not dict.__contains__(lab, "labels") else None
             if parts is not None:
                 self.opt.zero_grad(set_to_none=True)
-                loss = self.loss_fn.backward_from_parts(parts[0], parts[1], table, lab._index_fn())
+                with deferred_wgrads():
+                    loss = self.loss_fn.backward_from_parts(parts[0], parts[1], table, lab._index_fn())
         if loss is None:
             pred = self.model.forward_last(mfgs, val) if kind == "hidden" else val
             loss = _loss_backward(self.loss_fn, pred, mfgs[-1].dstdata["labels"], self.opt)
diff --git a/include/bliss_gnn.h b/include/bliss_gnn.h
--- a/include/bliss_gnn.h
+++ b/include/bliss_gnn.h
@@ -223,6 +223,9 @@
 } bliss_wgrad_t;
 int64_t bliss_sage_wgrad_workspace(const bliss_wgrad_t* probs, int32_t n_probs);
 int bliss_sage_wgrad(const bliss_wgrad_t* probs, int32_t n_probs, float* partials, int64_t partial_floats, void* stream);
+int64_t bliss_sage_wgrad_batch_workspace(const bliss_wgrad_t* probs, const int32_t* group_sizes, int32_t n_groups);
+int bliss_sage_wgrad_batch(const bliss_wgrad_t* probs, const int32_t* group_sizes, int32_t n_groups, float* partials,
+                           int64_t partial_floats, void* stream);
 
 int bliss_cross_entropy(const void* logits, int64_t stride, const int64_t* labels, int32_t n_rows, int32_t n_cls,
                         float* row_loss, void* dlogits, int64_t d_stride, float* loss_out, uint32_t* ticket, int32_t* err,
```
